# Jaureguy760/HaploHyped-VarAwareML

Hardware: AMD Instinct MI355X
Metric: variants/sec encode+compress, 3M-variant x 2.5k-sample VCF (higher is better)
Workload: dtype u8

## Files before the change

haplohyped_varawareml_amd/csrc/api.hip:

```cpp
#include "common.h"
#include <chrono>
#include <vector>
#include <stdarg.h>
#include <stdio.h>
#include <string.h>
#include <stdlib.h>

static thread_local char g_err[512] = "";

void hhgt_set_error(const char *fmt, ...)
{
    va_list ap;
    va_start(ap, fmt);
    vsnprintf(g_err, sizeof(g_err), fmt, ap);
    va_end(ap);
}

extern "C" const char *hhgt_last_error(void) { return g_err; }
extern "C" const char *hhgt_version(void) { return "hhgt 0.1 (gfx950)"; }

extern "C" int hhgt_device_count(void)
{
    int n = 0;
    if (hipGetDeviceCount(&n) != hipSuccess) return 0;
    return n;
}

int DevBuf::ensure(size_t bytes)
{
    if (bytes <= cap) return HHGT_OK;
    if (p) {
        hipFree(p);
        p = nullptr;
        cap = 0;
    }
    size_t want = bytes + bytes / 8 + 256;
    static const bool dbg = getenv("HHGT_ALLOC_DEBUG") != nullptr;
    const auto t0 = std::chrono::steady_clock::now();
    hipError_t e = hipMalloc(&p, want);
    if (dbg)
        fprintf(stderr, "[alloc] %.3f ms  hipMalloc %zu took %.3f ms\n", std::chrono::duration<double>(t0.time_since_epoch()).count() * 1e3,
                want, std::chrono::duration<double>(std::chrono::steady_clock::now() - t0).count() * 1e3);
    if (e != hipSuccess) {
        p = nullptr;
        hhgt_set_error("hipMalloc(%zu) failed: %s", want, hipGetErrorString(e));
        return HHGT_ERR_HIP;
    }
    cap = want;
    return HHGT_OK;
}

void DevBuf::release()
{
    if (p) hipFree(p);
    p = nullptr;
    cap = 0;
}

#define TRY(expr)                      \
    do {                               \
        int _rc = (expr);              \
        if (_rc != HHGT_OK) return _rc; \
    } while (0)

extern "C" int hhgt_ctx_create(int device, hhgt_ctx **out)
{
    if (!out) return HHGT_ERR_ARG;
    *out = nullptr;
    int n = hhgt_device_count();
    if (n <= 0 || device < 0 || device >= n) {
        hhgt_set_error("no usable HIP device (count=%d, requested=%d): libhhgt has no CPU path", n, device);
        return HHGT_ERR_NO_DEVICE;
    }
    HIP_TRY(hipSetDevice(device));
    hhgt_ctx *c = new hhgt_ctx();
    c->device = device;
    int rc = HHGT_OK;
    hipError_t e = hipGetDeviceProperties(&c->prop, device);
    if (e != hipSuccess) {
        hhgt_set_error("hipGetDeviceProperties failed: %s", hipGetErrorString(e));
        rc = HHGT_ERR_HIP;
    } else if (strncmp(c->prop.gcnArchName, "gfx950", 6) != 0) {
        hhgt_set_error("device %d is %s; libhhgt carries gfx950 code objects only", device, c->prop.gcnArchName);
        rc = HHGT_ERR_NO_DEVICE;
    }
    if (rc == HHGT_OK && (e = hipHostMalloc(reinterpret_cast<void **>(&c->h_counters), sizeof(DevCounters), hipHostMallocDefault)) != hipSuccess) {
        hhgt_set_error("hipHostMalloc failed: %s", hipGetErrorString(e));
        rc = HHGT_ERR_HIP;
    }
    if (rc == HHGT_OK && (e = hipHostMalloc(reinterpret_cast<void **>(&c->h_result_pinned), sizeof(hhgt_encode_result), hipHostMallocDefault)) != hipSuccess) {
        hhgt_set_error("hipHostMalloc failed: %s", hipGetErrorString(e));
        rc = HHGT_ERR_HIP;
    }
    if (rc == HHGT_OK) rc = c->counters.ensure(sizeof(DevCounters));
    if (rc != HHGT_OK) {
        hhgt_ctx_destroy(c);
        return rc;
    }
    *out = c;
    return HHGT_OK;
}

extern "C" void hhgt_ctx_destroy(hhgt_ctx *c)
{
    if (!c) return;
    hipSetDevice(c->device);
    hipDeviceSynchronize();
    DevBuf *bufs[] = {&c->slots, &c->counts, &c->prefix, &c->nl, &c->scan_tmp, &c->l_soff, &c->l_lend, &c->l_pos,
                      &c->l_refalt, &c->l_flags, &c->l_keep, &c->l_kidx, &c->l_cnew, &c->l_crun, &c->k_soff,
                      &c->k_lend, &c->k_meta, &c->redo_list, &c->redo_flag, &c->run_first, &c->run_names,
                      &c->counters, &c->cursor, &c->result, &c->dec_bad, &c->oh_ovl, &c->oh_lut, &c->crc_x2n};
    for (DevBuf *b : bufs) b->release();
    for (auto &w : c->cw) {
        DevBuf *wb[] = {&w.lz_scratch, &w.lz_csize, &w.lz_flags, &w.fr_bsize, &w.fr_csize, &w.fr_flags};
        for (DevBuf *b : wb) b->release();
        if (w.lz_done) hipEventDestroy(w.lz_done);
        if (w.fr_done) hipEventDestroy(w.fr_done);
    }
    if (c->h_counters) hipHostFree(c->h_counters);
    if (c->h_result_pinned) hipHostFree(c->h_result_pinned);
    for (auto &p : c->pending) {
        hipEventDestroy(p.a);
        hipEventDestroy(p.b);
    }
    for (auto e : c->event_pool) hipEventDestroy(e);
    delete c;
}

static hipEvent_t get_event(hhgt_ctx *c)
{
    if (!c->event_pool.empty()) {
        hipEvent_t e = c->event_pool.back();
        c->event_pool.pop_back();
        return e;
    }
    hipEvent_t e;
    hipEventCreate(&e);
    return e;
}

StageTimer::StageTimer(hhgt_ctx *c, hipStream_t s, int stage_) : ctx(c), st(s), stage(stage_)
{
    if (ctx->profiling) {
        a = get_event(ctx);
        b = get_event(ctx);
        hipEventRecord(a, st);
    }
}

void StageTimer::stop()
{
    if (a) {
        hipEventRecord(b, st);
        ctx->pending.push_back({stage, a, b});
        a = b = nullptr;
    }
}

int hhgt_profile_collect(hhgt_ctx *c)
{
    for (auto &p : c->pending) {
        hipEventSynchronize(p.b);
        float ms = 0.f;
        if (hipEventElapsedTime(&ms, p.a, p.b) == hipSuccess) {
            c->stage_ms[p.stage] += ms;
            c->stage_launches[p.stage] += 1;
        }
        c->event_pool.push_back(p.a);
        c->event_pool.push_back(p.b);
    }
    c->pending.clear();
    return HHGT_OK;
}

extern "C" int hhgt_profile_enable(hhgt_ctx *c, int on)
{
    if (!c) return HHGT_ERR_ARG;
    c->profiling = on ? 1 : 0;
    return HHGT_OK;
}

extern "C" int hhgt_profile_reset(hhgt_ctx *c)
{
    if (!c) return HHGT_ERR_ARG;
    hhgt_profile_collect(c);
    for (int i = 0; i < HHGT_N_STAGES; ++i) {
        c->stage_ms[i] = 0;
        c->stage_launches[i] = 0;
    }
    return HHGT_OK;
}

extern "C" int hhgt_profile_read(hhgt_ctx *c, double *ms, uint64_t *launches)
{
    if (!c) return HHGT_ERR_ARG;
    hhgt_profile_collect(c);
    for (int i = 0; i < HHGT_N_STAGES; ++i) {
        if (ms) ms[i] = c->stage_ms[i];
        if (launches) launches[i] = c->stage_launches[i];
    }
    return HHGT_OK;
}

static int make_layout(const hhgt_layout *lay, LayoutDev *L)
{
    if (!lay || lay->n_samples < 0) {
        hhgt_set_error("layout: bad n_samples");
        return HHGT_ERR_ARG;
    }
    L->S = (uint32_t)lay->n_samples;
    L->v_capacity = lay->v_capacity;
    L->ring = 0;
    L->pad_ = 0;
    if (lay->ring < 0 || (lay->ring > 0 && (lay->vc <= 0 || lay->v_capacity != (uint64_t)lay->ring * (uint64_t)lay->vc))) {
        hhgt_set_error("layout: a ring needs vc > 0 and v_capacity == ring * vc");
        return HHGT_ERR_ARG;
    }
    L->ring = (uint32_t)lay->ring;
    if (lay->vc == 0) {
        L->Vc = lay->v_capacity ? lay->v_capacity : TILE_V;
    } else {
        L->Vc = (uint64_t)lay->vc;
    }
    if (L->Vc % TILE_V) {
        hhgt_set_error("layout: variants per chunk (%llu) must be a multiple of %d (dense: v_capacity)",
                       (unsigned long long)L->Vc, TILE_V);
        return HHGT_ERR_ARG;
    }
    if (lay->v_capacity % L->Vc) {
        hhgt_set_error("layout: v_capacity must be a multiple of vc");
        return HHGT_ERR_ARG;
    }
    if (lay->sc == 0) {
        L->Sc = L->S ? L->S : 1;
        L->sc_log2 = 31;
        L->n_sc = 1;
    } else {
        uint32_t sc = (uint32_t)lay->sc;
        if (sc & (sc - 1)) {
            hhgt_set_error("layout: sc must be a power of two");
            return HHGT_ERR_ARG;
        }
        L->Sc = sc;
        uint32_t lg = 0;
        while ((1u << lg) < sc) ++lg;
        L->sc_log2 = lg;
        L->n_sc = (L->S + sc - 1) / sc;
        if (L->n_sc == 0) L->n_sc = 1;
    }
    return HHGT_OK;
}

extern "C" uint64_t hhgt_layout_bytes(const hhgt_layout *lay)
{
    LayoutDev L;
    if (make_layout(lay, &L) != HHGT_OK) return 0;
    return (uint64_t)L.n_sc * L.Sc * L.v_capacity * 2ull;
}

extern "C" uint64_t hhgt_layout_offset(const hhgt_layout *lay, uint32_t s, uint64_t v)
{
    LayoutDev L;
    if (make_layout(lay, &L) != HHGT_OK) return ~0ull;
    return layout_offset(L, s, v);
}

static int parse_region_host(const char *region, RegionFilter *rf)
{
    memset(rf, 0, sizeof(*rf));
    if (!region || !*region) return HHGT_OK;
    const char *colon = strrchr(region, ':');
    size_t clen = strlen(region);
    if (colon && colon[1] >= '0' && colon[1] <= '9') {
        char *p;
        long long b = strtoll(colon + 1, &p, 10), e = 0x7fffffffffffffffLL;
        while (*p == ',') p++;
        if (*p == '-' && p[1]) e = strtoll(p + 1, &p, 10);
        clen = (size_t)(colon - region);
        rf->has_range = 1;
        rf->beg = b;
        rf->end = e;
    }
    if (clen == 0 || clen >= sizeof(rf->contig)) {
        hhgt_set_error("region '%s': contig name empty or longer than 63 bytes", region);
        return HHGT_ERR_ARG;
    }
    memcpy(rf->contig, region, clen);
    rf->contig_len = (int)clen;
    return HHGT_OK;
}

__global__ void k_encode_finish(DevCounters *cnt, uint64_t *cursor, const uint64_t *__restrict__ run_first,
                                const uint8_t *__restrict__ run_names, uint64_t v_capacity, hhgt_encode_result *res)
{
    const uint32_t t = threadIdx.x;
    const uint64_t before = *cursor;
    const uint64_t kept = cnt->n_kept;
    __syncthreads();
    if (t == 0) {
        *cursor = before + kept;
        cnt->cursor_after = before + kept;
        res->stats.n_lines = cnt->n_lines;
        res->stats.n_records = cnt->n_records;
        res->stats.n_kept = kept;
        res->stats.n_drop_region = cnt->n_drop_region;
        res->stats.n_drop_filter = cnt->n_drop_filter;
        res->stats.n_haploid_padded = cnt->n_haploid;
        res->stats.n_malformed = cnt->n_malformed;
        res->stats.n_general_lines = cnt->n_general;
        res->stats.n_chrom_runs = cnt->n_chrom_runs;
        res->cursor_before = before;
        res->cursor_after = before + kept;
        res->n_lines_over = cnt->err_lines;
        res->err_density = cnt->err_density;
        res->v_capacity = v_capacity;
        res->done = 1u;
        res->reserved = cnt->n_other > 0xFFFFFFFFull ? 0xFFFFFFFFu : (uint32_t)cnt->n_other;
    }
    const uint64_t n_runs = cnt->n_chrom_runs;
    if (t < HHGT_RESULT_RUNS) res->run_first[t] = t < n_runs ? run_first[t] : 0ull;
    for (uint32_t q = t; q < HHGT_RESULT_RUNS * 32u; q += blockDim.x)
        res->run_names[q >> 5][q & 31u] = (q >> 5) < n_runs ? (char)run_names[q] : 0;
    __syncthreads();
    if (t < sizeof(DevCounters) / 8u) reinterpret_cast<unsigned long long *>(cnt)[t] = 0ull;
}

__global__ void k_set_u64(uint64_t *p, uint64_t v) { *p = v; }

static int encode_check_args(hhgt_ctx *c, const void *d_text, uint64_t nbytes, const hhgt_layout *lay, LayoutDev *L,
                             const char *region, RegionFilter *rf, void *d_G)
{
    TRY(make_layout(lay, L));
    if (nbytes >= 0xFFFFFFF0ull) {
        hhgt_set_error("encode: text block of %llu bytes; split it below 4 GiB at a line boundary",
                       (unsigned long long)nbytes);
        return HHGT_ERR_ARG;
    }
    if (nbytes && (!d_text || (reinterpret_cast<uintptr_t>(d_text) & 15u))) {
        hhgt_set_error("encode: d_text must be a 16-byte aligned device pointer");
        return HHGT_ERR_ARG;
    }
    if (L->S > 0 && !d_G) {
        hhgt_set_error("encode: d_G is NULL");
        return HHGT_ERR_ARG;
    }
    const int rc = parse_region_host(region, rf);
    rf->keep_multi = c->keep_multi;
    return rc;
}

static int encode_stage_index(hhgt_ctx *c, const uint8_t *text, uint64_t nbytes, uint32_t n_regions, uint32_t min_line, uint32_t S,
                              DevCounters *cnt, hipStream_t st)
{
    TRY(c->slots.ensure((size_t)n_regions * INDEX_CAP * 4));
    TRY(c->counts.ensure((size_t)n_regions * 4));
    TRY(c->prefix.ensure(((size_t)n_regions + 1) * 4));
    TRY(c->scan_tmp.ensure(2 * scan_tmp_elems(n_regions) * 4));
    TRY(launch_index_newlines(text, nbytes, c->slots.as<uint32_t>(), c->counts.as<uint32_t>(), n_regions, min_line, S, c->index_mode, cnt, st));
    TRY(launch_scan_exclusive_u32_pair(c->counts.as<uint32_t>(), c->prefix.as<uint32_t>(), nullptr, nullptr, n_regions,
                                       c->scan_tmp.as<uint32_t>(), c->scan_tmp.cap / 4, st));
    return HHGT_OK;
}

static int encode_stage_rest(hhgt_ctx *c, const uint8_t *text, uint64_t nbytes, uint32_t n_regions, uint32_t max_lines,
                             const RegionFilter &rf, const LayoutDev &L, const uint64_t *d_cursor, void *d_G, void *d_P, uint32_t *d_start, uint32_t *d_stop,
                             uint8_t *d_ref, uint8_t *d_alt, DevCounters *cnt, hipStream_t st)
{
    const uint32_t *d_nlines = c->prefix.as<uint32_t>() + n_regions;
    const size_t nl4 = ((size_t)max_lines + 1) * 4;
    TRY(c->nl.ensure(nl4));
    TRY(c->scan_tmp.ensure(2 * scan_tmp_elems(max_lines) * 4));
    DevBuf *per_line[] = {&c->l_soff, &c->l_lend, &c->l_pos, &c->l_refalt, &c->l_flags, &c->l_keep,
                          &c->l_kidx, &c->l_cnew, &c->l_crun, &c->k_soff, &c->k_lend, &c->k_meta,
                          &c->redo_list, &c->redo_flag};
    for (DevBuf *b : per_line) TRY(b->ensure(nl4));
    TRY(c->run_first.ensure(MAX_CHROM_RUNS * 8));
    TRY(c->run_names.ensure(MAX_CHROM_RUNS * 32));
    {
        StageTimer t(c, st, HHGT_STAGE_INDEX);
        TRY(launch_compact_newlines(c->slots.as<uint32_t>(), c->counts.as<uint32_t>(), c->prefix.as<uint32_t>(),
                                    n_regions, c->nl.as<uint32_t>(), max_lines, st));
        t.stop();
    }
    if (max_lines == 0) return HHGT_OK;
    {
        StageTimer t(c, st, HHGT_STAGE_FIXED);
        TRY(launch_parse_fixed(text, nbytes, c->nl.as<uint32_t>(), d_nlines, max_lines, rf, L.S,
                               c->l_soff.as<uint32_t>(), c->l_lend.as<uint32_t>(), c->l_pos.as<uint32_t>(),
                               c->l_refalt.as<uint32_t>(), c->l_flags.as<uint32_t>(), c->l_keep.as<uint32_t>(),
                               c->l_cnew.as<uint32_t>(), c->index_mode, cnt, st));
        TRY(launch_scan_exclusive_u32_pair(c->l_keep.as<uint32_t>(), c->l_kidx.as<uint32_t>(), c->l_cnew.as<uint32_t>(),
                                           c->l_crun.as<uint32_t>(), max_lines, c->scan_tmp.as<uint32_t>(), c->scan_tmp.cap / 4, st));
        TRY(launch_compact_kept(text, nbytes, c->nl.as<uint32_t>(), d_nlines, max_lines, c->l_soff.as<uint32_t>(),
                                c->l_lend.as<uint32_t>(), c->l_pos.as<uint32_t>(), c->l_refalt.as<uint32_t>(),
                                c->l_flags.as<uint32_t>(), c->l_kidx.as<uint32_t>(), c->l_crun.as<uint32_t>(),
                                c->k_soff.as<uint32_t>(), c->k_lend.as<uint32_t>(), c->k_meta.as<uint32_t>(),
                                c->redo_list.as<uint32_t>(), c->redo_flag.as<uint32_t>(), c->run_first.as<uint64_t>(), c->run_names.as<uint8_t>(),
                                MAX_CHROM_RUNS, d_cursor, L.v_capacity, L.ring, d_start, d_stop, d_ref, d_alt, cnt, d_P != nullptr, st));
        t.stop();
    }
    if (L.S > 0) {
        StageTimer t(c, st, HHGT_STAGE_ENCODE);
        if (d_P)
            TRY(launch_encode_planes(text, nbytes, c->k_soff.as<uint32_t>(), c->k_meta.as<uint32_t>(), max_lines, d_cursor, L,
                                     static_cast<uint8_t *>(d_P), static_cast<int8_t *>(d_G), c->redo_list.as<uint32_t>(),
                                     c->redo_flag.as<uint32_t>(), cnt, st));
        else
            TRY(launch_encode_tiles(text, nbytes, c->k_soff.as<uint32_t>(), c->k_meta.as<uint32_t>(), max_lines, d_cursor,
                                    L, static_cast<int8_t *>(d_G), c->redo_list.as<uint32_t>(),
                                    c->redo_flag.as<uint32_t>(), cnt, st));
        t.stop();
        StageTimer t2(c, st, HHGT_STAGE_GENERAL);
        TRY(launch_encode_general(text, nbytes, c->k_soff.as<uint32_t>(), c->k_lend.as<uint32_t>(),
                                  c->k_meta.as<uint32_t>(), c->redo_list.as<uint32_t>(), d_cursor, L,
                                  static_cast<int8_t *>(d_G), static_cast<uint8_t *>(d_P), cnt, c->prop.multiProcessorCount, st));
        t2.stop();
    }
    return HHGT_OK;
}

static int encode_finish(hhgt_ctx *c, uint64_t *d_cursor, const LayoutDev &L, DevCounters *cnt, hipStream_t st)
{
    TRY(c->run_first.ensure(MAX_CHROM_RUNS * 8));
    TRY(c->run_names.ensure(MAX_CHROM_RUNS * 32));
    TRY(c->result.ensure(sizeof(hhgt_encode_result)));
    hipLaunchKernelGGL(k_encode_finish, dim3(1), dim3(256), 0, st, cnt, d_cursor, c->run_first.as<uint64_t>(),
                       c->run_names.as<uint8_t>(), L.ring ? 0ull : L.v_capacity, c->result.as<hhgt_encode_result>());
    HIP_TRY(hipGetLastError());
    return HHGT_OK;
}

extern "C" int hhgt_encode_result_status(const hhgt_encode_result *r)
{
    if (!r) return HHGT_ERR_ARG;
    if (!r->done) {
        hhgt_set_error("encode: the result record is not complete yet (synchronise the stream first)");
        return HHGT_ERR_ARG;
    }
    if (r->err_density) {
        hhgt_set_error("encode: more than %u newlines inside one %u-byte region (not VCF text)", INDEX_CAP, INDEX_REGION);
        return HHGT_ERR_LINE_DENSITY;
    }
    if (r->n_lines_over) {
        hhgt_set_error("encode: %llu lines beyond max_lines were not encoded", (unsigned long long)r->n_lines_over);
        return HHGT_ERR_CAPACITY;
    }
    if (r->stats.n_malformed) {
        hhgt_set_error("Error parsing VCF file: %llu malformed record(s) (too few columns, bad POS, FORMAT without GT)",
                       (unsigned long long)r->stats.n_malformed);
        return HHGT_ERR_MALFORMED;
    }
    if (r->v_capacity && r->cursor_after > r->v_capacity) {
        hhgt_set_error("encode: %llu kept records at v_base %llu exceed v_capacity %llu",
                       (unsigned long long)r->stats.n_kept, (unsigned long long)r->cursor_before,
                       (unsigned long long)r->v_capacity);
        return HHGT_ERR_CAPACITY;
    }
    if (r->stats.n_chrom_runs > MAX_CHROM_RUNS) {
        hhgt_set_error("encode: %llu CHROM runs in one text block, more than the limit of %u (a run starts at every change of CHROM "
                       "and behind every empty or header line)",
                       (unsigned long long)r->stats.n_chrom_runs, MAX_CHROM_RUNS);
        return HHGT_ERR_CAPACITY;
    }
    return HHGT_OK;
}

static void empty_result(hhgt_encode_result *r)
{
    memset(r, 0, sizeof(*r));
    r->done = 1u;
}

static int planes_check_layout(const LayoutDev &L)
{
    if (L.Vc % 4096ull) {
        hhgt_set_error("planes: variants per chunk (%llu; dense: v_capacity) must be a multiple of 4096", (unsigned long long)L.Vc);
        return HHGT_ERR_ARG;
    }
    return HHGT_OK;
}

extern "C" uint64_t hhgt_planes_bytes(const hhgt_layout *lay)
{
    LayoutDev L;
    if (make_layout(lay, &L) != HHGT_OK || planes_check_layout(L) != HHGT_OK) return 0;
    return (uint64_t)L.n_sc * L.Sc * L.v_capacity / 2ull;
}

static int planes_columns(const hhgt_layout *lay, uint32_t col0, uint32_t n_cols, LayoutDev *L, PlanesGeom *pg)
{
    TRY(make_layout(lay, L));
    TRY(planes_check_layout(*L));
    if ((uint64_t)col0 + n_cols > L->v_capacity / L->Vc) {
        hhgt_set_error("planes: columns [%u, %u) outside the layout's %llu", col0, col0 + n_cols, (unsigned long long)(L->v_capacity / L->Vc));
        return HHGT_ERR_ARG;
    }
    *pg = planes_geom(*L, col0);
    return HHGT_OK;
}

static int encode_async_impl(hhgt_ctx *c, const void *d_text, uint64_t nbytes, const char *region, const hhgt_layout *lay,
                             uint64_t *d_cursor, uint32_t max_lines, void *d_G, void *d_P, bool planes, uint32_t *d_start,
                             uint32_t *d_stop, uint8_t *d_ref, uint8_t *d_alt, hhgt_encode_result *h_result, void *stream)
{
    if (!c || !d_cursor) return HHGT_ERR_ARG;
    hipStream_t st = reinterpret_cast<hipStream_t>(stream);
    HIP_TRY(hipSetDevice(c->device));
    LayoutDev L;
    RegionFilter rf;
    TRY(encode_check_args(c, d_text, nbytes, lay, &L, region, &rf, planes ? d_P : d_G));
    if (planes) TRY(planes_check_layout(L));
    const uint8_t *text = static_cast<const uint8_t *>(d_text);
    DevCounters *cnt = c->counters.as<DevCounters>();
    if (!c->counters_clean) HIP_TRY(hipMemsetAsync(cnt, 0, sizeof(DevCounters), st));
    c->counters_clean = false;
    const uint32_t n_regions = (uint32_t)((nbytes + 1 + INDEX_REGION - 1) / INDEX_REGION);
    if (nbytes) {
        {
            StageTimer t(c, st, HHGT_STAGE_INDEX);
            TRY(encode_stage_index(c, text, nbytes, n_regions, L.S ? 2u * L.S + 17u : 0u, L.S, cnt, st));
            t.stop();
        }
        TRY(encode_stage_rest(c, text, nbytes, n_regions, max_lines, rf, L, d_cursor, d_G, planes ? d_P : nullptr, d_start, d_stop, d_ref,
                              d_alt, cnt, st));
    }
    TRY(encode_finish(c, d_cursor, L, cnt, st));
    c->counters_clean = true;
    if (h_result) {
        h_result->done = 0u;
        HIP_TRY(hipMemcpyAsync(h_result, c->result.p, sizeof(hhgt_encode_result), hipMemcpyDeviceToHost, st));
    }
    return HHGT_OK;
}

extern "C" int hhgt_encode_text_async(hhgt_ctx *c, const void *d_text, uint64_t nbytes, const char *region,
                                      const hhgt_layout *lay, uint64_t *d_cursor, uint32_t max_lines, void *d_G,
                                      uint32_t *d_start, uint32_t *d_stop, uint8_t *d_ref, uint8_t *d_alt,
                                      hhgt_encode_result *h_result, void *stream)
{
    return encode_async_impl(c, d_text, nbytes, region, lay, d_cursor, max_lines, d_G, nullptr, false, d_start, d_stop, d_ref, d_alt,
                             h_result, stream);
}

extern "C" int hhgt_encode_text_planes_async(hhgt_ctx *c, const void *d_text, uint64_t nbytes, const char *region,
                                             const hhgt_layout *lay, uint64_t *d_cursor, uint32_t max_lines, void *d_P, void *d_G,
                                             uint32_t *d_start, uint32_t *d_stop, uint8_t *d_ref, uint8_t *d_alt,
                                             hhgt_encode_result *h_result, void *stream)
{
    return encode_async_impl(c, d_text, nbytes, region, lay, d_cursor, max_lines, d_G, d_P, true, d_start, d_stop, d_ref, d_alt,
                             h_result, stream);
}

extern "C" int hhgt_pad_tail_planes(hhgt_ctx *c, const hhgt_layout *lay, uint64_t v_end, uint64_t vcol_begin, uint64_t vcol_end,
                                    void *d_P, void *stream)
{
    if (!c || !d_P) return HHGT_ERR_ARG;
    HIP_TRY(hipSetDevice(c->device));
    LayoutDev L;
    TRY(make_layout(lay, &L));
    TRY(planes_check_layout(L));
    if (v_end > L.v_capacity || vcol_end > L.v_capacity / L.Vc) {
        hhgt_set_error("pad_tail: range outside the layout");
        return HHGT_ERR_ARG;
    }
    return launch_pad_tail_planes(L, v_end, vcol_begin, vcol_end, static_cast<uint8_t *>(d_P), reinterpret_cast<hipStream_t>(stream));
}

extern "C" int hhgt_pad_tail_planes_cursor(hhgt_ctx *c, const hhgt_layout *lay, const uint64_t *d_cursor, void *d_P, void *stream)
{
    if (!c || !d_P || !d_cursor) return HHGT_ERR_ARG;
    HIP_TRY(hipSetDevice(c->device));
    LayoutDev L;
    TRY(make_layout(lay, &L));
    TRY(planes_check_layout(L));
    return launch_pad_tail_planes_cursor(L, d_cursor, static_cast<uint8_t *>(d_P), reinterpret_cast<hipStream_t>(stream));
}

extern "C" int hhgt_planes_expand(hhgt_ctx *c, const hhgt_layout *lay, const void *d_P, const void *d_G, uint32_t col0, uint32_t n_cols,
                                  void *d_out, void *stream)
{
    if (!c || !d_P || !d_out) return HHGT_ERR_ARG;
    HIP_TRY(hipSetDevice(c->device));
    LayoutDev L;
    PlanesGeom pg;
    TRY(planes_columns(lay, col0, n_cols, &L, &pg));
    if (n_cols == 0) return HHGT_OK;
    return launch_planes_expand(L, static_cast<const uint8_t *>(d_P), static_cast<const uint8_t *>(d_G), col0, n_cols,
                                static_cast<uint8_t *>(d_out), reinterpret_cast<hipStream_t>(stream));
}

static int encode_text_once(hhgt_ctx *c, const void *d_text, uint64_t nbytes, const char *region, const hhgt_layout *lay, uint64_t v_base,
                            void *d_G, uint32_t *d_start, uint32_t *d_stop, uint8_t *d_ref, uint8_t *d_alt, hhgt_encode_stats *stats,
                            void *stream);

extern "C" int hhgt_encode_text(hhgt_ctx *c, const void *d_text, uint64_t nbytes, const char *region,
                                const hhgt_layout *lay, uint64_t v_base, void *d_G, uint32_t *d_start,
                                uint32_t *d_stop, uint8_t *d_ref, uint8_t *d_alt, hhgt_encode_stats *stats,
                                void *stream)
{
    int rc = encode_text_once(c, d_text, nbytes, region, lay, v_base, d_G, d_start, d_stop, d_ref, d_alt, stats, stream);
    if (rc == HHGT_ERR_MALFORMED && c && lay && lay->n_samples >= 760) {
        const int mode = c->index_mode < 0 ? index_mode_default() : c->index_mode;
        if (mode > 0) {
            const int saved = c->index_mode;
            c->index_mode = 0;
            rc = encode_text_once(c, d_text, nbytes, region, lay, v_base, d_G, d_start, d_stop, d_ref, d_alt, stats, stream);
            c->index_mode = saved;
        }
    }
    return rc;
}

static int encode_text_once(hhgt_ctx *c, const void *d_text, uint64_t nbytes, const char *region, const hhgt_layout *lay, uint64_t v_base,
                            void *d_G, uint32_t *d_start, uint32_t *d_stop, uint8_t *d_ref, uint8_t *d_alt, hhgt_encode_stats *stats,
                            void *stream)
{
    if (!c) return HHGT_ERR_ARG;
    hipStream_t st = reinterpret_cast<hipStream_t>(stream);
    HIP_TRY(hipSetDevice(c->device));
    if (stats) memset(stats, 0, sizeof(*stats));
    LayoutDev L;
    RegionFilter rf;
    TRY(encode_check_args(c, d_text, nbytes, lay, &L, region, &rf, d_G));
    c->run_first_kept.clear();
    c->run_names_host.clear();
    if (nbytes == 0) return HHGT_OK;

    const uint8_t *text = static_cast<const uint8_t *>(d_text);
    DevCounters *cnt = c->counters.as<DevCounters>();
    TRY(c->cursor.ensure(8));
    HIP_TRY(hipMemsetAsync(cnt, 0, sizeof(DevCounters), st));
    c->counters_clean = false;
    hipLaunchKernelGGL(k_set_u64, dim3(1), dim3(1), 0, st, c->cursor.as<uint64_t>(), v_base);
    const uint32_t n_regions = (uint32_t)((nbytes + 1 + INDEX_REGION - 1) / INDEX_REGION);
    uint32_t n_lines = 0;
    {
        StageTimer t(c, st, HHGT_STAGE_INDEX);
        TRY(encode_stage_index(c, text, nbytes, n_regions, L.S ? 2u * L.S + 17u : 0u, L.S, cnt, st));
        c->h_counters->n_lines = 0;
        c->h_counters->err_density = 0;
        HIP_TRY(hipMemcpyAsync(&c->h_counters->n_lines, c->prefix.as<uint32_t>() + n_regions, 4,
                               hipMemcpyDeviceToHost, st));
        HIP_TRY(hipMemcpyAsync(&c->h_counters->err_density, &cnt->err_density, 8, hipMemcpyDeviceToHost, st));
        HIP_TRY(hipStreamSynchronize(st));
        t.stop();
        n_lines = (uint32_t)(c->h_counters->n_lines & 0xFFFFFFFFull);
        if (c->h_counters->err_density) {
            hhgt_set_error("encode: more than %u newlines inside one %u-byte region (not VCF text)", INDEX_CAP,
                           INDEX_REGION);
            return HHGT_ERR_LINE_DENSITY;
        }
    }
    if (stats) stats->n_lines = n_lines;
    if (n_lines == 0) return HHGT_OK;
    TRY(encode_stage_rest(c, text, nbytes, n_regions, n_lines, rf, L, c->cursor.as<uint64_t>(), d_G, nullptr, d_start, d_stop, d_ref,
                          d_alt, cnt, st));
    TRY(encode_finish(c, c->cursor.as<uint64_t>(), L, cnt, st));
    c->counters_clean = true;
    hhgt_encode_result *hr = &c->h_result;
    hr->done = 0u;
    HIP_TRY(hipMemcpyAsync(c->h_result_pinned, c->result.p, sizeof(hhgt_encode_result), hipMemcpyDeviceToHost, st));
    HIP_TRY(hipStreamSynchronize(st));
    *hr = *c->h_result_pinned;
    if (stats) *stats = hr->stats;
    TRY(hhgt_encode_result_status(hr));
    const uint32_t n_runs = (uint32_t)hr->stats.n_chrom_runs;
    if (n_runs) {
        std::vector<uint64_t> first(n_runs);
        std::vector<char> names((size_t)n_runs * 32);
        if (n_runs <= HHGT_RESULT_RUNS) {
            memcpy(first.data(), hr->run_first, n_runs * 8);
            memcpy(names.data(), hr->run_names, (size_t)n_runs * 32);
        } else {
            HIP_TRY(hipMemcpy(first.data(), c->run_first.p, (size_t)n_runs * 8, hipMemcpyDeviceToHost));
            HIP_TRY(hipMemcpy(names.data(), c->run_names.p, (size_t)n_runs * 32, hipMemcpyDeviceToHost));
        }
        for (uint32_t r = 0; r < n_runs; ++r) {
            c->run_first_kept.push_back(first[r]);
            c->run_names_host.emplace_back(names.data() + (size_t)r * 32, strnlen(names.data() + (size_t)r * 32, 31));
        }
    }
    return HHGT_OK;
}

extern "C" int hhgt_encode_chrom_runs(hhgt_ctx *c, uint32_t max_runs, uint64_t *first_kept, char *names,
                                      uint32_t *n_runs)
{
    if (!c || !n_runs) return HHGT_ERR_ARG;
    uint32_t n = (uint32_t)c->run_first_kept.size();
    *n_runs = n;
    if (n > max_runs) n = max_runs;
    for (uint32_t r = 0; r < n; ++r) {
        if (first_kept) first_kept[r] = c->run_first_kept[r];
        if (names) {
            memset(names + (size_t)r * 32, 0, 32);
            size_t l = c->run_names_host[r].size() < 31 ? c->run_names_host[r].size() : 31;
            memcpy(names + (size_t)r * 32, c->run_names_host[r].data(), l);
        }
    }
    return HHGT_OK;
}

extern "C" int hhgt_pad_tail(hhgt_ctx *c, const hhgt_layout *lay, uint64_t v_end, uint64_t vcol_begin,
                             uint64_t vcol_end, void *d_G, void *stream)
{
    if (!c || !d_G) return HHGT_ERR_ARG;
    HIP_TRY(hipSetDevice(c->device));
    LayoutDev L;
    TRY(make_layout(lay, &L));
    if (v_end > L.v_capacity || vcol_end > L.v_capacity / L.Vc) {
        hhgt_set_error("pad_tail: range outside the layout");
        return HHGT_ERR_ARG;
    }
    return launch_pad_tail(L, v_end, vcol_begin, vcol_end, static_cast<int8_t *>(d_G),
                           reinterpret_cast<hipStream_t>(stream));
}

extern "C" int hhgt_pad_tail_cursor(hhgt_ctx *c, const hhgt_layout *lay, const uint64_t *d_cursor, void *d_G, void *stream)
{
    if (!c || !d_G || !d_cursor) return HHGT_ERR_ARG;
    HIP_TRY(hipSetDevice(c->device));
    LayoutDev L;
    TRY(make_layout(lay, &L));
    return launch_pad_tail_cursor(L, d_cursor, static_cast<int8_t *>(d_G), reinterpret_cast<hipStream_t>(stream));
}

static int check_codec_args(uint64_t chunk_nbytes, int typesize, int blocksize, int format)
{
    if (typesize < 1 || typesize > 255 || blocksize < 16 || blocksize > 65536 || blocksize % typesize ||
        chunk_nbytes == 0 || chunk_nbytes >= 0x7fffffffull || (format != HHGT_BLOSC1 && format != HHGT_BLOSC2)) {
        hhgt_set_error("compress: bad arguments (chunk_nbytes=%llu typesize=%d blocksize=%d format=%d)",
                       (unsigned long long)chunk_nbytes, typesize, blocksize, format);
        return HHGT_ERR_ARG;
    }
    return HHGT_OK;
}

static int effective_blocksize(uint64_t chunk_nbytes, int typesize, int blocksize)
{
    if ((uint64_t)blocksize > chunk_nbytes) {
        blocksize = (int)chunk_nbytes;
        if (typesize > 1 && blocksize >= typesize) blocksize -= blocksize % typesize;
    }
    return blocksize > 0 ? blocksize : 1;
}

static int check_decode_block(int typesize, int blocksize)
{
    if (blocksize > 65536) {
        hhgt_set_error("decode: block of %d bytes x typesize %d does not fit LDS (blocks of at most 65536 bytes)",
                       blocksize, typesize);
        return HHGT_ERR_ARG;
    }
    return HHGT_OK;
}

static void codec_geometry(uint64_t chunk_nbytes, int typesize, int blocksize, uint32_t *nblocks, uint32_t *nwaves,
                           size_t *slot_bytes)
{
    const bool split = typesize >= 2 && typesize <= 16 && blocksize / typesize >= 128;
    *nblocks = (uint32_t)((chunk_nbytes + blocksize - 1) / blocksize);
    *nwaves = split ? (uint32_t)typesize : 1u;
    size_t max_stream = split ? (size_t)blocksize / typesize : (size_t)blocksize;
    if (split && chunk_nbytes % blocksize && chunk_nbytes % blocksize > max_stream) max_stream = chunk_nbytes % blocksize;
    *slot_bytes = lz4_slot_bytes((int)max_stream);
}

extern "C" uint64_t hhgt_compress_bound(uint64_t n_chunks, uint64_t chunk_nbytes, int typesize, int blocksize)
{
    if (check_codec_args(chunk_nbytes, typesize, blocksize, HHGT_BLOSC2) != HHGT_OK) return 0;
    return n_chunks * (chunk_nbytes + 32);
}

static int compress_impl(hhgt_ctx *c, const void *d_src, const void *d_planes, PlanesGeom pg, uint64_t n_chunks, uint64_t chunk_nbytes,
                         int typesize, int blocksize, int format, void *d_dst, uint64_t dst_cap,
                         uint64_t *d_chunk_off, uint64_t *total_bytes, void *stream)
{
    if (!c || (!d_src && !d_planes) || !d_dst || !d_chunk_off) return HHGT_ERR_ARG;
    hipStream_t st = reinterpret_cast<hipStream_t>(stream);
    HIP_TRY(hipSetDevice(c->device));
    TRY(check_codec_args(chunk_nbytes, typesize, blocksize, format));
    if (total_bytes) *total_bytes = 0;
    if (n_chunks == 0) return HHGT_OK;
    if (!total_bytes && dst_cap < n_chunks * (chunk_nbytes + 32)) {
        hhgt_set_error("compress: the asynchronous form (total_bytes == NULL) needs dst_cap >= hhgt_compress_bound() = %llu, got %llu",
                       (unsigned long long)(n_chunks * (chunk_nbytes + 32)), (unsigned long long)dst_cap);
        return HHGT_ERR_CAPACITY;
    }
    blocksize = effective_blocksize(chunk_nbytes, typesize, blocksize);
    uint32_t nblocks, nwaves;
    size_t slot;
    codec_geometry(chunk_nbytes, typesize, blocksize, &nblocks, &nwaves, &slot);
    const uint64_t n_streams = n_chunks * nblocks * nwaves;
    hipStream_t fst = c->frame_stream ? c->frame_stream : st;
    hhgt_ctx::CodecWs &w = c->cw[c->frame_stream ? (c->cmp_seq++ & 1u) : 0u];
    TRY(w.lz_scratch.ensure((size_t)n_streams * slot));
    TRY(w.lz_csize.ensure((size_t)n_streams * 4));
    TRY(w.fr_bsize.ensure((size_t)n_chunks * nblocks * 4));
    TRY(w.fr_csize.ensure(((size_t)n_chunks + 1) * 8));
    TRY(w.fr_flags.ensure((size_t)n_chunks * 4));
    if (w.fr_pending) {
        HIP_TRY(hipStreamWaitEvent(st, w.fr_done, 0));
        w.fr_pending = false;
    }
    {
        StageTimer t(c, st, HHGT_STAGE_LZ4);
        if (!w.lz_flags.p) {
            TRY(w.lz_flags.ensure(4));
            HIP_TRY(hipMemsetAsync(w.lz_flags.p, 0, 4, st));
        }
        if (++w.lz_tag == 0) w.lz_tag = 1;
        TRY(launch_lz4_blocks(static_cast<const uint8_t *>(d_src), static_cast<const uint8_t *>(d_planes), pg, n_chunks, chunk_nbytes, typesize,
                              blocksize, w.lz_scratch.as<uint8_t>(), slot, w.lz_csize.as<uint32_t>(), c->clevel, w.lz_flags.as<uint32_t>(),
                              w.lz_tag, st));
        t.stop();
    }
    if (fst != st) {
        if (!w.lz_done) HIP_TRY(hipEventCreateWithFlags(&w.lz_done, hipEventDisableTiming));
        if (!w.fr_done) HIP_TRY(hipEventCreateWithFlags(&w.fr_done, hipEventDisableTiming));
        HIP_TRY(hipEventRecord(w.lz_done, st));
        HIP_TRY(hipStreamWaitEvent(fst, w.lz_done, 0));
    }
    {
        StageTimer t(c, fst, HHGT_STAGE_FRAME);
        TRY(launch_frame(w.lz_scratch.as<uint8_t>(), slot, w.lz_csize.as<uint32_t>(),
                         static_cast<const uint8_t *>(d_src), static_cast<const uint8_t *>(d_planes), pg, n_chunks, chunk_nbytes, typesize,
                         blocksize, format, w.fr_bsize.as<uint32_t>(), w.fr_csize.as<uint64_t>(), static_cast<uint8_t *>(d_dst),
                         dst_cap, d_chunk_off, w.fr_flags.as<uint32_t>(), fst));
        t.stop();
    }
    if (fst != st) {
        HIP_TRY(hipEventRecord(w.fr_done, fst));
        w.fr_pending = true;
        if (total_bytes) HIP_TRY(hipStreamWaitEvent(st, w.fr_done, 0));
    }
    if (total_bytes) {
        uint64_t tot = 0;
        HIP_TRY(hipMemcpyAsync(&tot, d_chunk_off + n_chunks, 8, hipMemcpyDeviceToHost, st));
        HIP_TRY(hipStreamSynchronize(st));
        *total_bytes = tot;
        if (tot > dst_cap) {
            hhgt_set_error("compress: need %llu bytes, dst_cap is %llu", (unsigned long long)tot,
                           (unsigned long long)dst_cap);
            return HHGT_ERR_CAPACITY;
        }
    }
    return HHGT_OK;
}

extern "C" int hhgt_compress_chunks(hhgt_ctx *c, const void *d_src, uint64_t n_chunks, uint64_t chunk_nbytes,
                                    int typesize, int blocksize, int format, void *d_dst, uint64_t dst_cap,
                                    uint64_t *d_chunk_off, uint64_t *total_bytes, void *stream)
{
    if (!d_src) return HHGT_ERR_ARG;
    return compress_impl(c, d_src, nullptr, PlanesGeom{0, 0, 0, 0}, n_chunks, chunk_nbytes, typesize, blocksize, format, d_dst, dst_cap,
                         d_chunk_off, total_bytes, stream);
}

extern "C" int hhgt_compress_planes(hhgt_ctx *c, const hhgt_layout *lay, const void *d_P, const void *d_G, uint32_t col0, uint32_t n_cols,
                                    int format, void *d_dst, uint64_t dst_cap, uint64_t *d_chunk_off, uint64_t *total_bytes,
                                    void *stream)
{
    if (!c || !d_P) return HHGT_ERR_ARG;
    LayoutDev L;
    PlanesGeom pg;
    TRY(planes_columns(lay, col0, n_cols, &L, &pg));
    const uint64_t chunk_nbytes = (uint64_t)L.Sc * L.Vc * 2ull, col_bytes = chunk_nbytes * L.n_sc;
    const uint8_t *g = d_G ? static_cast<const uint8_t *>(d_G) + (uint64_t)col0 * col_bytes : nullptr;
    return compress_impl(c, g, d_P, pg, (uint64_t)n_cols * L.n_sc, chunk_nbytes, 2, 8192, format, d_dst, dst_cap, d_chunk_off, total_bytes,
                         stream);
}

extern "C" int hhgt_reserve(hhgt_ctx *c, uint64_t text_bytes, uint32_t max_lines, uint64_t n_chunks, uint64_t chunk_nbytes, int typesize,
                            int blocksize)
{
    if (!c) return HHGT_ERR_ARG;
    HIP_TRY(hipSetDevice(c->device));
    if (text_bytes) {
        const uint32_t n_regions = (uint32_t)((text_bytes + 1 + INDEX_REGION - 1) / INDEX_REGION);
        TRY(c->slots.ensure((size_t)n_regions * INDEX_CAP * 4));
        TRY(c->counts.ensure((size_t)n_regions * 4));
        TRY(c->prefix.ensure(((size_t)n_regions + 1) * 4));
        const size_t st_el = scan_tmp_elems(n_regions) > scan_tmp_elems(max_lines) ? scan_tmp_elems(n_regions) : scan_tmp_elems(max_lines);
        TRY(c->scan_tmp.ensure(2 * st_el * 4));
        const size_t nl4 = ((size_t)max_lines + 1) * 4;
        TRY(c->nl.ensure(nl4));
        DevBuf *per_line[] = {&c->l_soff, &c->l_lend, &c->l_pos, &c->l_refalt, &c->l_flags, &c->l_keep, &c->l_kidx, &c->l_cnew, &c->l_crun,
                              &c->k_soff, &c->k_lend, &c->k_meta, &c->redo_list, &c->redo_flag};
        for (DevBuf *b : per_line) TRY(b->ensure(nl4));
        TRY(c->run_first.ensure(MAX_CHROM_RUNS * 8));
        TRY(c->run_names.ensure(MAX_CHROM_RUNS * 32));
        TRY(c->result.ensure(sizeof(hhgt_encode_result)));
    }
    if (n_chunks) {
        TRY(check_codec_args(chunk_nbytes, typesize, blocksize, HHGT_BLOSC2));
        blocksize = effective_blocksize(chunk_nbytes, typesize, blocksize);
        uint32_t nblocks, nwaves;
        size_t slot;
        codec_geometry(chunk_nbytes, typesize, blocksize, &nblocks, &nwaves, &slot);
        const uint64_t n_streams = n_chunks * nblocks * nwaves;
        hhgt_ctx::CodecWs &w = c->cw[0];
        TRY(w.lz_scratch.ensure((size_t)n_streams * slot));
        TRY(w.lz_csize.ensure((size_t)n_streams * 4));
        TRY(w.fr_bsize.ensure((size_t)n_chunks * nblocks * 4));
        TRY(w.fr_csize.ensure(((size_t)n_chunks + 1) * 8));
        TRY(w.fr_flags.ensure((size_t)n_chunks * 4));
    }
    return HHGT_OK;
}

extern "C" int hhgt_set_clevel(hhgt_ctx *c, int clevel)
{
    if (!c || clevel < 1 || clevel > 9) {
        hhgt_set_error("clevel must be 1..9");
        return HHGT_ERR_ARG;
    }
    c->clevel = clevel;
    return HHGT_OK;
}

extern "C" int hhgt_stream_create(hhgt_ctx *c, int kind, void **out)
{
    if (!c || !out || (kind != HHGT_STREAM_ENCODE && kind != HHGT_STREAM_COMPRESS && kind != HHGT_STREAM_FRAME)) {
        hhgt_set_error("hhgt_stream_create: bad arguments");
        return HHGT_ERR_ARG;
    }
    HIP_TRY(hipSetDevice(c->device));
    hipStream_t st = nullptr;
    if (kind == HHGT_STREAM_FRAME) {
        HIP_TRY(hipStreamCreateWithFlags(&st, hipStreamNonBlocking));
    } else if (kind == HHGT_STREAM_ENCODE) {
        int lo = 0, hi = 0;
        HIP_TRY(hipDeviceGetStreamPriorityRange(&lo, &hi));
        HIP_TRY(hipStreamCreateWithPriority(&st, hipStreamNonBlocking, hi));
    } else {
        const uint32_t n_cu = (uint32_t)c->prop.multiProcessorCount;
        uint32_t use = n_cu >= 128u ? (n_cu * 3u / 4u) / 32u * 32u : n_cu;
        if (const char *e = getenv("HHGT_COMPRESS_CUS")) {
            const int v = atoi(e);
            use = v <= 0 || (uint32_t)v >= n_cu ? n_cu : (uint32_t)v;
        }
        if (use >= n_cu) {
            HIP_TRY(hipStreamCreateWithFlags(&st, hipStreamNonBlocking));
        } else {
            std::vector<uint32_t> mask((n_cu + 31u) / 32u, 0u);
            for (uint32_t i = n_cu - use; i < n_cu; ++i) mask[i >> 5] |= 1u << (i & 31u);
            if (hipExtStreamCreateWithCUMask(&st, (uint32_t)mask.size(), mask.data()) != hipSuccess) {
                (void)hipGetLastError();
                st = nullptr;
                HIP_TRY(hipStreamCreateWithFlags(&st, hipStreamNonBlocking));
            }
        }
    }
    *out = st;
    return HHGT_OK;
}

extern "C" int hhgt_set_frame_stream(hhgt_ctx *c, void *stream)
{
    if (!c) return HHGT_ERR_ARG;
    HIP_TRY(hipSetDevice(c->device));
    if (c->frame_stream) HIP_TRY(hipStreamSynchronize(c->frame_stream));
    for (auto &w : c->cw) w.fr_pending = false;
    c->frame_stream = reinterpret_cast<hipStream_t>(stream);
    return HHGT_OK;
}

extern "C" int hhgt_stream_destroy(hhgt_ctx *c, void *stream)
{
    if (!c) return HHGT_ERR_ARG;
    if (stream) {
        HIP_TRY(hipSetDevice(c->device));
        if (reinterpret_cast<hipStream_t>(stream) == c->frame_stream) TRY(hhgt_set_frame_stream(c, nullptr));
        HIP_TRY(hipStreamDestroy(reinterpret_cast<hipStream_t>(stream)));
    }
    return HHGT_OK;
}

extern "C" int hhgt_set_index_mode(hhgt_ctx *c, int mode)
{
    if (!c || mode < -1 || mode > 2) {
        hhgt_set_error("index mode must be -1 (default), 0 (scan), 1 (hop) or 2 (walk)");
        return HHGT_ERR_ARG;
    }
    c->index_mode = mode;
    return HHGT_OK;
}

extern "C" int hhgt_set_keep_multiallelic(hhgt_ctx *c, int on)
{
    if (!c) return HHGT_ERR_ARG;
    c->keep_multi = on ? 1 : 0;
    return HHGT_OK;
}

__global__ void k_count_nonzero_u32(const uint32_t *__restrict__ v, uint64_t n, unsigned long long *out)
{
    uint64_t i = (uint64_t)blockIdx.x * blockDim.x + threadIdx.x;
    const unsigned long long m = __ballot(i < n && v[i] != 0u);
    if ((threadIdx.x & 63u) == 0u && m) atomicAdd(out, (unsigned long long)__builtin_popcountll(m));
}

extern "C" int hhgt_inflate_members(hhgt_ctx *c, const void *d_src, uint64_t src_bytes, const uint64_t *d_comp_off,
                                    const uint32_t *d_comp_len, const uint64_t *d_out_off, const uint32_t *d_isize,
                                    uint64_t n_members, void *d_dst, uint64_t dst_bytes, const uint32_t *d_crc32,
                                    uint32_t *d_status, uint64_t *n_bad, void *stream)
{
    if (!c || !d_src || !d_comp_off || !d_comp_len || !d_out_off || !d_isize || !d_status || (!d_dst && dst_bytes))
        return HHGT_ERR_ARG;
    hipStream_t st = reinterpret_cast<hipStream_t>(stream);
    HIP_TRY(hipSetDevice(c->device));
    if (n_bad) *n_bad = 0;
    if (n_members == 0) return HHGT_OK;
    if (d_crc32 && !c->crc_x2n_ready) {
        uint32_t t[32];
        crc32_x2n_table(t);
        TRY(c->crc_x2n.ensure(sizeof(t)));
        HIP_TRY(hipMemcpy(c->crc_x2n.p, t, sizeof(t), hipMemcpyHostToDevice));
        c->crc_x2n_ready = true;
    }
    {
        StageTimer t(c, st, HHGT_STAGE_INFLATE);
        TRY(launch_inflate(static_cast<const uint8_t *>(d_src), src_bytes, d_comp_off, d_comp_len, d_out_off, d_isize,
                           n_members, static_cast<uint8_t *>(d_dst), dst_bytes, d_status, d_crc32,
                           c->crc_x2n.as<uint32_t>(), st));
        t.stop();
    }
    if (n_bad) {
        TRY(c->dec_bad.ensure(8));
        HIP_TRY(hipMemsetAsync(c->dec_bad.p, 0, 8, st));
        hipLaunchKernelGGL(k_count_nonzero_u32, dim3((uint32_t)((n_members + 255) / 256)), dim3(256), 0, st, d_status,
                           n_members, c->dec_bad.as<unsigned long long>());
        HIP_TRY(hipGetLastError());
        uint64_t nb = 0;
        HIP_TRY(hipMemcpyAsync(&nb, c->dec_bad.p, 8, hipMemcpyDeviceToHost, st));
        HIP_TRY(hipStreamSynchronize(st));
        *n_bad = nb;
    }
    return HHGT_OK;
}

extern "C" int hhgt_decompress_chunks(hhgt_ctx *c, const void *d_src, const uint64_t *d_chunk_off, uint64_t n_chunks,
                                      uint64_t chunk_nbytes, int typesize, int blocksize, void *d_dst,
                                      uint64_t *n_bad, void *stream)
{
    if (!c || !d_src || !d_dst || !d_chunk_off) return HHGT_ERR_ARG;
    hipStream_t st = reinterpret_cast<hipStream_t>(stream);
    HIP_TRY(hipSetDevice(c->device));
    TRY(check_decode_block(typesize, blocksize));
    TRY(check_codec_args(chunk_nbytes, typesize, blocksize, HHGT_BLOSC2));
    if (n_bad) *n_bad = 0;
    if (n_chunks == 0) return HHGT_OK;
    blocksize = effective_blocksize(chunk_nbytes, typesize, blocksize);
    TRY(c->dec_bad.ensure(8));
    HIP_TRY(hipMemsetAsync(c->dec_bad.p, 0, 8, st));
    {
        StageTimer t(c, st, HHGT_STAGE_DECODE);
        TRY(launch_decode(static_cast<const uint8_t *>(d_src), d_chunk_off, n_chunks, chunk_nbytes, typesize,
                          blocksize, static_cast<uint8_t *>(d_dst), c->dec_bad.as<unsigned long long>(), st));
        t.stop();
    }
    if (n_bad) {
        uint64_t nb = 0;
        HIP_TRY(hipMemcpyAsync(&nb, c->dec_bad.p, 8, hipMemcpyDeviceToHost, st));
        HIP_TRY(hipStreamSynchronize(st));
        *n_bad = nb;
    }
    return HHGT_OK;
}

extern "C" int hhgt_decompress_blocks(hhgt_ctx *c, const hhgt_block_sel *d_sel, uint32_t n_sel, uint64_t chunk_nbytes,
                                      int typesize, int blocksize, void *d_dst, uint64_t *n_bad, void *stream)
{
    if (!c || (n_sel && (!d_sel || !d_dst))) {
        hhgt_set_error("decompress_blocks: null %s", !c ? "context" : !d_sel ? "selection array" : "destination");
        return HHGT_ERR_ARG;
    }
    hipStream_t st = reinterpret_cast<hipStream_t>(stream);
    HIP_TRY(hipSetDevice(c->device));
    TRY(check_decode_block(typesize, blocksize));
    TRY(check_codec_args(chunk_nbytes, typesize, blocksize, HHGT_BLOSC2));
    if (n_bad) *n_bad = 0;
    if (n_sel == 0) return HHGT_OK;
    blocksize = effective_blocksize(chunk_nbytes, typesize, blocksize);
    TRY(c->dec_bad.ensure(8));
    HIP_TRY(hipMemsetAsync(c->dec_bad.p, 0, 8, st));
    {
        StageTimer t(c, st, HHGT_STAGE_DECODE);
        TRY(launch_decode_sel(d_sel, n_sel, chunk_nbytes, typesize, blocksize, static_cast<uint8_t *>(d_dst),
                              c->dec_bad.as<unsigned long long>(), st));
        t.stop();
    }
    if (n_bad) {
        uint64_t nb = 0;
        HIP_TRY(hipMemcpyAsync(&nb, c->dec_bad.p, 8, hipMemcpyDeviceToHost, st));
        HIP_TRY(hipStreamSynchronize(st));
        *n_bad = nb;
    }
    return HHGT_OK;
}

extern "C" int hhgt_count_alleles(hhgt_ctx *c, const hhgt_count_sel *d_sel, uint32_t n_sel, uint32_t sc, uint32_t vc,
                                  int typesize, int blocksize, uint32_t *d_counts, uint64_t n_out, uint64_t *n_bad,
                                  void *stream)
{
    if (!c || (n_sel && (!d_sel || !d_counts))) {
        hhgt_set_error("count_alleles: null %s", !c ? "context" : !d_sel ? "selection array" : "counts");
        return HHGT_ERR_ARG;
    }
    if (typesize != 2) {
        hhgt_set_error("count_alleles: typesize %d (only 2: one diploid int8 call)", typesize);
        return HHGT_ERR_ARG;
    }
    if (sc < 1 || sc > 64 || vc < 1) {
        hhgt_set_error("count_alleles: chunk of %u samples x %u variants (1 to 64 samples)", sc, vc);
        return HHGT_ERR_ARG;
    }
    const uint64_t chunk_nbytes = (uint64_t)sc * vc * 2u;
    TRY(check_codec_args(chunk_nbytes, typesize, blocksize, HHGT_BLOSC2));
    if (blocksize > 8192 || ((uint64_t)vc * 2u) % (uint64_t)blocksize) {
        hhgt_set_error("count_alleles: blocksize %d does not cut a row of %u variants into whole blocks of at most 8192 "
                       "bytes", blocksize, vc);
        return HHGT_ERR_ARG;
    }
    hipStream_t st = reinterpret_cast<hipStream_t>(stream);
    HIP_TRY(hipSetDevice(c->device));
    if (n_bad) *n_bad = 0;
    if (n_sel == 0) return HHGT_OK;
    TRY(c->dec_bad.ensure(8));
    HIP_TRY(hipMemsetAsync(c->dec_bad.p, 0, 8, st));
    {
        StageTimer t(c, st, HHGT_STAGE_DECODE);
        TRY(launch_count_alleles(d_sel, n_sel, sc, vc, blocksize, d_counts, n_out, c->dec_bad.as<unsigned long long>(), st));
        t.stop();
    }
    if (n_bad) {
        uint64_t nb = 0;
        HIP_TRY(hipMemcpyAsync(&nb, c->dec_bad.p, 8, hipMemcpyDeviceToHost, st));
        HIP_TRY(hipStreamSynchronize(st));
        *n_bad = nb;
    }
    return HHGT_OK;
}

extern "C" int hhgt_count_samples(hhgt_ctx *c, const hhgt_sample_sel *d_sel, uint32_t n_sel, uint32_t sc, uint32_t vc,
                                  int typesize, int blocksize, const uint32_t *d_vmask, uint64_t vmask_words,
                                  uint32_t *d_counts, uint64_t n_out, uint64_t *n_bad, void *stream)
{
    if (!c || (n_sel && (!d_sel || !d_counts))) {
        hhgt_set_error("count_samples: null %s", !c ? "context" : !d_sel ? "selection array" : "counts");
        return HHGT_ERR_ARG;
    }
    if (typesize != 2) {
        hhgt_set_error("count_samples: typesize %d (only 2: one diploid int8 call)", typesize);
        return HHGT_ERR_ARG;
    }
    if (sc < 1 || sc > 64 || vc < 1) {
        hhgt_set_error("count_samples: chunk of %u samples x %u variants (1 to 64 samples)", sc, vc);
        return HHGT_ERR_ARG;
    }
    const uint64_t chunk_nbytes = (uint64_t)sc * vc * 2u;
    TRY(check_codec_args(chunk_nbytes, typesize, blocksize, HHGT_BLOSC2));
    if (blocksize > 8192 || ((uint64_t)vc * 2u) % (uint64_t)blocksize) {
        hhgt_set_error("count_samples: blocksize %d does not cut a row of %u variants into whole blocks of at most 8192 "
                       "bytes", blocksize, vc);
        return HHGT_ERR_ARG;
    }
    hipStream_t st = reinterpret_cast<hipStream_t>(stream);
    HIP_TRY(hipSetDevice(c->device));
    if (n_bad) *n_bad = 0;
    if (n_sel == 0) return HHGT_OK;
    TRY(c->dec_bad.ensure(8));
    HIP_TRY(hipMemsetAsync(c->dec_bad.p, 0, 8, st));
    {
        StageTimer t(c, st, HHGT_STAGE_DECODE);
        TRY(launch_count_samples(d_sel, n_sel, sc, vc, blocksize, d_vmask, vmask_words, d_counts, n_out,
                                 c->dec_bad.as<unsigned long long>(), st));
        t.stop();
    }
    if (n_bad) {
        uint64_t nb = 0;
        HIP_TRY(hipMemcpyAsync(&nb, c->dec_bad.p, 8, hipMemcpyDeviceToHost, st));
        HIP_TRY(hipStreamSynchronize(st));
        *n_bad = nb;
    }
    return HHGT_OK;
}
```

haplohyped_varawareml_amd/csrc/common.h:

```cpp
#pragma once
#include <hip/hip_runtime.h>
#include <stdint.h>
#include <stddef.h>
#include <string>
#include <vector>
#include "../../include/hhgt.h"

#define HHGT_WAVE 64
#ifdef HHGT_ENC_PRIO
#define HHGT_WAVE_PRIO() __builtin_amdgcn_s_setprio(HHGT_ENC_PRIO)
#else
#define HHGT_WAVE_PRIO()
#endif

#ifdef __HIPCC__
__device__ __forceinline__ uint32_t wave_scan_sum_dpp(uint32_t x, uint32_t lane)
{
    x += (uint32_t)__builtin_amdgcn_update_dpp(0, (int)x, 0x111, 0xf, 0xf, false);
    x += (uint32_t)__builtin_amdgcn_update_dpp(0, (int)x, 0x112, 0xf, 0xf, false);
    x += (uint32_t)__builtin_amdgcn_update_dpp(0, (int)x, 0x114, 0xf, 0xf, false);
    x += (uint32_t)__builtin_amdgcn_update_dpp(0, (int)x, 0x118, 0xf, 0xf, false);
    const uint32_t t0 = (uint32_t)__builtin_amdgcn_readlane((int)x, 15);
    const uint32_t t1 = (uint32_t)__builtin_amdgcn_readlane((int)x, 31) + t0;
    const uint32_t t2 = (uint32_t)__builtin_amdgcn_readlane((int)x, 47) + t1;
    const uint32_t row = lane >> 4;
    return x + (row == 0u ? 0u : (row == 1u ? t0 : (row == 2u ? t1 : t2)));
}
#endif

void hhgt_set_error(const char *fmt, ...);
#define HIP_TRY(expr)                                                                      \
    do {                                                                                   \
        hipError_t _e = (expr);                                                            \
        if (_e != hipSuccess) {                                                            \
            hhgt_set_error("%s failed: %s (%s:%d)", #expr, hipGetErrorString(_e), __FILE__, \
                           __LINE__);                                                      \
            return HHGT_ERR_HIP;                                                           \
        }                                                                                  \
    } while (0)

enum : uint32_t {
    LF_RECORD = 1u,
    LF_KEEP = 2u,
    LF_FAST = 4u,
    LF_MALFORMED = 8u,
    LF_DROP_REGION = 16u,
    LF_DROP_FILTER = 32u,
    LF_CHROM_NEW = 64u,
};

struct DevCounters {
    unsigned long long n_lines;
    unsigned long long n_records;
    unsigned long long n_kept;
    unsigned long long n_drop_region;
    unsigned long long n_drop_filter;
    unsigned long long n_haploid;
    unsigned long long n_malformed;
    unsigned long long n_general;
    unsigned long long n_chrom_runs;
    unsigned long long err_density;
    unsigned long long err_lines;
    unsigned long long cursor_after;
    unsigned long long n_other;
    unsigned long long pad[3];
};

#define MAX_CHROM_RUNS 4096u

struct RegionFilter {
    char contig[64];
    int contig_len;
    int has_range;
    long long beg, end;
    int keep_multi;
};

#define INDEX_REGION 16384u
#define INDEX_CAP 1024u

#define TILE_V 128
#define TILE_S 256

struct LayoutDev {
    uint32_t S;
    uint32_t sc_log2;
    uint32_t n_sc;
    uint32_t Sc;
    uint64_t Vc;
    uint64_t v_capacity;
    uint32_t ring;
    uint32_t pad_;
};

#define PL_TILE 256u
struct PlanesGeom {
    uint32_t S_pad;
    uint32_t bpr;
    uint32_t tpc;
    uint32_t col0;
};
static inline __host__ __device__ uint64_t planes_piece(const PlanesGeom &g, uint64_t col, uint32_t tile, uint32_t kp, uint32_t row)
{
    return ((((col * g.tpc + tile) * 4ull + kp) * g.S_pad) + row) * 32ull;
}
static inline __host__ __device__ PlanesGeom planes_geom(const LayoutDev &L, uint32_t col0)
{
    PlanesGeom g;
    g.S_pad = L.n_sc * L.Sc;
    g.bpr = (uint32_t)(L.Vc >> 12);
    g.tpc = (uint32_t)(L.Vc / PL_TILE);
    g.col0 = col0;
    return g;
}
static inline __host__ __device__ void planes_block(const PlanesGeom &g, uint64_t id, uint64_t *col, uint32_t *row, uint32_t *bi)
{
    const uint64_t per_col = (uint64_t)g.S_pad * g.bpr;
    const uint64_t c = id / per_col;
    const uint32_t rem = (uint32_t)(id - c * per_col);
    *col = g.col0 + c;
    *row = rem / g.bpr;
    *bi = rem - (rem / g.bpr) * g.bpr;
}

struct DevBuf {
    void *p = nullptr;
    size_t cap = 0;
    int ensure(size_t bytes);
    void release();
    template <typename T> T *as() const { return reinterpret_cast<T *>(p); }
};

struct hhgt_ctx {
    int device = 0;
    hipDeviceProp_t prop;
    DevBuf slots, counts, prefix, nl, scan_tmp;
    DevBuf l_soff, l_lend, l_pos, l_refalt, l_flags, l_keep, l_kidx, l_cnew, l_crun;
    DevBuf k_soff, k_lend, k_meta, redo_list, redo_flag, run_first, run_names;
    DevBuf counters;
    DevBuf cursor;
    DevBuf result;
    struct CodecWs {
        DevBuf lz_scratch, lz_csize, lz_flags, fr_bsize, fr_csize, fr_flags;
        uint32_t lz_tag = 0;
        hipEvent_t lz_done = nullptr, fr_done = nullptr;
        bool fr_pending = false;
    } cw[2];
    uint64_t cmp_seq = 0;
    hipStream_t frame_stream = nullptr;
    DevBuf dec_bad, oh_ovl, oh_lut, crc_x2n;
    bool crc_x2n_ready = false;
    DevCounters *h_counters = nullptr;
    hhgt_encode_result *h_result_pinned = nullptr;
    hhgt_encode_result h_result;
    std::vector<uint64_t> run_first_kept;
    std::vector<std::string> run_names_host;
    int clevel = 5;
    int keep_multi = 0;
    int index_mode = -1;
    bool counters_clean = false;
    int profiling = 0;
    double stage_ms[HHGT_N_STAGES] = {0};
    uint64_t stage_launches[HHGT_N_STAGES] = {0};
    struct Pending { int stage; hipEvent_t a, b; };
    std::vector<Pending> pending;
    std::vector<hipEvent_t> event_pool;
};

struct StageTimer {
    hhgt_ctx *ctx;
    hipStream_t st;
    int stage;
    hipEvent_t a = nullptr, b = nullptr;
    StageTimer(hhgt_ctx *c, hipStream_t s, int stage_);
    void stop();
};
int hhgt_profile_collect(hhgt_ctx *ctx);

int launch_scan_exclusive_u32(const uint32_t *d_in, uint32_t *d_out, uint64_t n, uint32_t *d_tmp,
                              size_t tmp_elems, hipStream_t st);
int launch_scan_exclusive_u32_pair(const uint32_t *in_a, uint32_t *out_a, const uint32_t *in_b, uint32_t *out_b, uint64_t n,
                                   uint32_t *d_tmp, size_t tmp_elems, hipStream_t st);
size_t scan_tmp_elems(uint64_t n);

int launch_index_newlines(const uint8_t *d_text, uint64_t n, uint32_t *d_slots, uint32_t *d_counts,
                          uint32_t n_regions, uint32_t min_line, uint32_t S, int mode, DevCounters *d_cnt, hipStream_t st);
int index_mode_default();
int launch_compact_newlines(const uint32_t *d_slots, const uint32_t *d_counts, const uint32_t *d_prefix,
                            uint32_t n_regions, uint32_t *d_nl, uint32_t max_lines, hipStream_t st);
int launch_parse_fixed(const uint8_t *d_text, uint64_t n, const uint32_t *d_nl, const uint32_t *d_nlines,
                       uint32_t max_lines, const RegionFilter &region, uint32_t S, uint32_t *l_soff, uint32_t *l_lend,
                       uint32_t *l_pos, uint32_t *l_refalt, uint32_t *l_flags, uint32_t *l_keep,
                       uint32_t *l_cnew, int mode, DevCounters *d_cnt, hipStream_t st);
int launch_compact_kept(const uint8_t *d_text, uint64_t n, const uint32_t *d_nl, const uint32_t *d_nlines, uint32_t max_lines,
                        const uint32_t *l_soff, const uint32_t *l_lend,
                        const uint32_t *l_pos, const uint32_t *l_refalt, const uint32_t *l_flags,
                        const uint32_t *l_kidx, const uint32_t *l_crun, uint32_t *k_soff, uint32_t *k_lend,
                        uint32_t *k_meta, uint32_t *redo_list, uint32_t *redo_flag, uint64_t *run_first, uint8_t *run_names,
                        uint32_t max_runs, const uint64_t *d_cursor, uint64_t v_capacity, uint32_t ring, uint32_t *d_start,
                        uint32_t *d_stop, uint8_t *d_ref, uint8_t *d_alt, DevCounters *d_cnt, bool strided, hipStream_t st);

int launch_encode_tiles(const uint8_t *d_text, uint64_t n, const uint32_t *k_soff, const uint32_t *k_meta,
                        uint32_t n_lines_bound, const uint64_t *d_cursor, LayoutDev lay, int8_t *d_G,
                        uint32_t *redo_list, uint32_t *redo_flag, DevCounters *d_cnt, hipStream_t st);
int launch_encode_general(const uint8_t *d_text, uint64_t n, const uint32_t *k_soff, const uint32_t *k_lend,
                          const uint32_t *k_meta, const uint32_t *redo_list, const uint64_t *d_cursor, LayoutDev lay,
                          int8_t *d_G, uint8_t *d_P, DevCounters *d_cnt, int n_cu, hipStream_t st);
int launch_encode_planes(const uint8_t *d_text, uint64_t n, const uint32_t *k_soff, const uint32_t *k_meta,
                         uint32_t n_lines_bound, const uint64_t *d_cursor, LayoutDev lay, uint8_t *d_P, int8_t *d_G,
                         uint32_t *redo_list, uint32_t *redo_flag, DevCounters *d_cnt, hipStream_t st);
int launch_pad_tail_planes(LayoutDev lay, uint64_t v_end, uint64_t vcol_begin, uint64_t vcol_end, uint8_t *d_P, hipStream_t st);
int launch_pad_tail_planes_cursor(LayoutDev lay, const uint64_t *d_cursor, uint8_t *d_P, hipStream_t st);
int launch_planes_expand(LayoutDev lay, const uint8_t *d_P, const uint8_t *d_G, uint32_t col0, uint32_t n_cols, uint8_t *d_out, hipStream_t st);
int launch_pad_tail(LayoutDev lay, uint64_t v_end, uint64_t vcol_begin, uint64_t vcol_end, int8_t *d_G,
                    hipStream_t st);
int launch_pad_tail_cursor(LayoutDev lay, const uint64_t *d_cursor, int8_t *d_G, hipStream_t st);

size_t lz4_slot_bytes(int neblock);
int launch_lz4_blocks(const uint8_t *d_src, const uint8_t *d_planes, PlanesGeom pg, uint64_t n_chunks, uint64_t chunk_nbytes, int typesize,
                      int blocksize, uint8_t *d_scratch, size_t slot_bytes, uint32_t *d_csize, int clevel, uint32_t *d_flags, uint32_t tag,
                      hipStream_t st);
int launch_lz4_bitplanes(const uint8_t *d_src, bool planes, PlanesGeom pg, uint64_t n_blocks, uint8_t *d_scratch, size_t slot_bytes, uint32_t *d_csize,
                         int depth, uint32_t *d_flags, uint32_t tag, hipStream_t st);
int launch_frame(const uint8_t *d_scratch, size_t slot_bytes, const uint32_t *d_csize, const uint8_t *d_src, const uint8_t *d_planes,
                 PlanesGeom pg, uint64_t n_chunks, uint64_t chunk_nbytes, int typesize, int blocksize, int format,
                 uint32_t *d_bstart, uint64_t *d_chunk_csize, uint8_t *d_dst, uint64_t dst_cap,
                 uint64_t *d_chunk_off, uint32_t *d_chunk_flags, hipStream_t st);
int launch_decode(const uint8_t *d_src, const uint64_t *d_chunk_off, uint64_t n_chunks, uint64_t chunk_nbytes,
                  int typesize, int blocksize, uint8_t *d_dst, unsigned long long *d_bad, hipStream_t st);
int launch_decode_sel(const hhgt_block_sel *d_sel, uint32_t n_sel, uint64_t chunk_nbytes, int typesize, int blocksize,
                      uint8_t *d_dst, unsigned long long *d_bad, hipStream_t st);
int launch_count_alleles(const hhgt_count_sel *d_sel, uint32_t n_sel, uint32_t sc, uint32_t vc, int blocksize,
                         uint32_t *d_counts, uint64_t n_out, unsigned long long *d_bad, hipStream_t st);
int launch_count_samples(const hhgt_sample_sel *d_sel, uint32_t n_sel, uint32_t sc, uint32_t vc, int blocksize,
                         const uint32_t *d_vmask, uint64_t vmask_words, uint32_t *d_counts, uint64_t n_out,
                         unsigned long long *d_bad, hipStream_t st);
int launch_inflate(const uint8_t *d_src, uint64_t src_bytes, const uint64_t *d_comp_off, const uint32_t *d_comp_len,
                   const uint64_t *d_out_off, const uint32_t *d_isize, uint64_t n_members, uint8_t *d_dst,
                   uint64_t dst_bytes, uint32_t *d_status, const uint32_t *d_crc32, const uint32_t *d_x2n, hipStream_t st);
void crc32_x2n_table(uint32_t *t );

static inline __host__ __device__ uint64_t layout_offset(const LayoutDev &L, uint32_t s, uint64_t v)
{
    uint64_t vcol = v / L.Vc, vin = v - vcol * L.Vc;
    if (L.ring) vcol %= L.ring;
    uint32_t scol = (L.sc_log2 >= 31) ? 0u : (s >> L.sc_log2);
    uint32_t sin = s - scol * L.Sc;
    return (((vcol * L.n_sc + scol) * L.Sc + sin) * L.Vc + vin) * 2ull;
}
```

haplohyped_varawareml_amd/csrc/index.hip:

```cpp
#include "common.h"

typedef uint32_t u32x4_unaligned __attribute__((ext_vector_type(4), aligned(1)));
typedef uint32_t u32x4_t __attribute__((ext_vector_type(4)));

__device__ __forceinline__ uint32_t nl_mask4(uint32_t x)
{
    uint32_t t = x ^ 0x0A0A0A0Au;
    uint32_t z = ~(((t & 0x7F7F7F7Fu) + 0x7F7F7F7Fu) | t | 0x7F7F7F7Fu);
    return (((z >> 7) * 0x01020408u) >> 24) & 0xFu;
}

__global__ __launch_bounds__(256) void k_index_newlines(const uint8_t *__restrict__ text, uint64_t n,
                                                        uint32_t *__restrict__ slots,
                                                        uint32_t *__restrict__ counts, uint32_t n_regions,
                                                        DevCounters *cnt)
{
    HHGT_WAVE_PRIO();
    const uint32_t lane = threadIdx.x & 63u;
    const uint32_t r = blockIdx.x * 4u + (threadIdx.x >> 6);
    if (r >= n_regions) return;
    const bool virt = n > 0 && text[n - 1] != '\n';
    const uint64_t rbase = (uint64_t)r * INDEX_REGION;
    uint32_t *my = slots + (size_t)r * INDEX_CAP;
    uint32_t wcount = 0;
    bool overflow = false;
    uint32_t masks[INDEX_REGION / 1024];
#pragma unroll
    for (int it = 0; it < (int)(INDEX_REGION / 1024); ++it) {
        uint64_t g0 = rbase + (uint64_t)it * 1024u + lane * 16u;
        uint32_t m = 0;
        if (g0 + 16 <= n) {
            const u32x4_t v4 = __builtin_nontemporal_load(reinterpret_cast<const u32x4_t *>(text + g0));
            uint4 v = make_uint4(v4.x, v4.y, v4.z, v4.w);
            m = nl_mask4(v.x) | (nl_mask4(v.y) << 4) | (nl_mask4(v.z) << 8) | (nl_mask4(v.w) << 12);
        } else if (g0 <= n) {
            for (int j = 0; j < 16; ++j) {
                uint64_t g = g0 + j;
                if (g < n) {
                    if (text[g] == '\n') m |= 1u << j;
                } else if (g == n && virt)
                    m |= 1u << j;
            }
        }
        masks[it] = m;
    }
#pragma unroll
    for (int it = 0; it < (int)(INDEX_REGION / 1024); ++it) {
        uint32_t m = masks[it];
        if (__ballot(m != 0) == 0ull) continue;
        uint32_t c = __popc(m);
        uint32_t inc = c;
#pragma unroll
        for (int d = 1; d < 64; d <<= 1) {
            uint32_t t = __shfl_up(inc, d, 64);
            if (lane >= (uint32_t)d) inc += t;
        }
        uint32_t idx = wcount + inc - c;
        uint32_t g0 = (uint32_t)(rbase + (uint64_t)it * 1024u + lane * 16u);
        while (m) {
            int j = __ffs(m) - 1;
            m &= m - 1;
            if (idx < INDEX_CAP) my[idx] = g0 + (uint32_t)j;
            else overflow = true;
            ++idx;
        }
        wcount += __shfl(inc, 63, 64);
    }
    if (__ballot(overflow) != 0ull && lane == 0) atomicAdd(&cnt->err_density, 1ull);
    if (lane == 0) counts[r] = wcount < INDEX_CAP ? wcount : INDEX_CAP;
}

__device__ __forceinline__ uint32_t eq_mask4(uint32_t x, uint32_t c4)
{
    const uint32_t t = x ^ c4;
    const uint32_t z = ~(((t & 0x7F7F7F7Fu) + 0x7F7F7F7Fu) | t | 0x7F7F7F7Fu);
    return (((z >> 7) * 0x01020408u) >> 24) & 0xFu;
}

__device__ __forceinline__ uint32_t eq_mask16(const u32x4_t &v, uint32_t c4)
{
    return eq_mask4(v.x, c4) | (eq_mask4(v.y, c4) << 4) | (eq_mask4(v.z, c4) << 8) | (eq_mask4(v.w, c4) << 12);
}

__device__ __forceinline__ uint32_t head_byte(const u32x4_t &v, uint32_t off)
{
    const uint32_t q = (off >> 2) & 3u;
    const uint32_t d = q == 0u ? v.x : (q == 1u ? v.y : (q == 2u ? v.z : v.w));
    return ((uint32_t)__builtin_amdgcn_readlane((int)d, (int)(off >> 4)) >> (8u * (off & 3u))) & 0xFFu;
}

__device__ __forceinline__ uint32_t head_kth(uint32_t m16, uint32_t cum, uint32_t k)
{
    const unsigned long long b = __builtin_amdgcn_ballot_w64(cum < k && cum + (uint32_t)__popc(m16) >= k);
    const int l = __builtin_ctzll(b);
    uint32_t m = (uint32_t)__builtin_amdgcn_readlane((int)m16, l);
    const uint32_t r = k - (uint32_t)__builtin_amdgcn_readlane((int)cum, l);
    for (uint32_t i = 1; i < r; ++i) m &= m - 1u;
    return 16u * (uint32_t)l + (uint32_t)__builtin_ctz(m);
}

#ifndef WALK_BATCH
#define WALK_BATCH 1
#endif
#ifndef WALK_PF
#define WALK_PF 0
#endif
template <int U, bool WALK>
__global__ __launch_bounds__(256) void k_index_hop(const uint8_t *__restrict__ text, uint64_t n, uint32_t *__restrict__ slots,
                                                   uint32_t *__restrict__ counts, uint32_t n_regions, uint32_t skip, uint32_t S,
                                                   DevCounters *cnt, uint32_t HOP_K)
{
    HHGT_WAVE_PRIO();
    const uint32_t lane = threadIdx.x & 63u;
    const uint32_t w = (uint32_t)__builtin_amdgcn_readfirstlane((int)(blockIdx.x * 4u + (threadIdx.x >> 6)));
    const uint32_t r_first = w * HOP_K;
    if (r_first >= n_regions) return;
    const uint32_t r_cnt = n_regions - r_first < HOP_K ? n_regions - r_first : HOP_K;
    const bool virt = n > 0 && text[n - 1] != '\n';
    const uint64_t beg = (uint64_t)r_first * INDEX_REGION;
    uint64_t endw = beg + (uint64_t)r_cnt * INDEX_REGION;
    if (endw > n + 1) endw = n + 1;
    const uint64_t last_term = virt ? n : n - 1;
    uint32_t cntv = 0;
    bool overflow = false;
    uint64_t pos = beg;
    uint64_t cand = 0, fb = 0;
    bool have_cand = false;
    uint64_t est_len = 0, pf_wb = 0;
    bool pf_valid = false;
    u32x4_t pf = u32x4_t{0u, 0u, 0u, 0u};
    auto record = [&](uint64_t q) {
        const uint32_t rr = (uint32_t)(q / INDEX_REGION), local = rr - r_first;
        const uint32_t c = (uint32_t)__builtin_amdgcn_readlane((int)cntv, (int)local);
        if (c < INDEX_CAP) {
            if (lane == 0) slots[(size_t)rr * INDEX_CAP + c] = (uint32_t)q;
        } else
            overflow = true;
        cntv += lane == local ? 1u : 0u;
    };
    bool no_batch = false, bat_off = false;
    uint32_t bat_fail = 0;
    uint64_t head_p = 0;
    bool cand_batch = false;
    bool rehead = false;
    while (have_cand || pos < endw) {
        if (WALK && WALK_BATCH && have_cand && !no_batch && !bat_off && est_len != 0ull && cand >= 40ull && cand + 3ull * est_len + 216ull <= n) {
            const uint32_t g = lane >> 4, li = lane & 15u;
            const uint64_t L0 = est_len;
            const uint8_t *wbase = text + (cand - 40ull);
            const uint64_t voff = (uint64_t)g * L0 + 16ull * li;
            const u32x4_t v = *reinterpret_cast<const u32x4_unaligned *>(wbase + voff);
            const uint32_t nlm = eq_mask16(v, 0x0A0A0A0Au), tbm = eq_mask16(v, 0x09090909u);
            const unsigned long long nlb = __builtin_amdgcn_ballot_w64(nlm != 0u);
            uint32_t og[4];
            bool vg[4];
#pragma unroll
            for (int k = 0; k < 4; ++k) {
                const uint32_t mg = (uint32_t)(nlb >> (16 * k)) & 0xFFFFu;
                vg[k] = mg != 0u;
                const int fl = 16 * k + __builtin_ctz(mg | 0x10000u);
                og[k] = 16u * ((uint32_t)fl & 15u) + (uint32_t)__builtin_ctz((uint32_t)__builtin_amdgcn_readlane((int)nlm, fl & 63) | 0x10000u);
            }
            const uint32_t o = g == 0u ? og[0] : (g == 1u ? og[1] : (g == 2u ? og[2] : og[3]));
            const uint32_t l0 = 16u * li;
            const uint32_t keep = l0 > o ? 0xFFFFu : (l0 + 15u <= o ? 0u : (0xFFFFu << (o - l0 + 1u)) & 0xFFFFu);
            const unsigned long long nl2 = __builtin_amdgcn_ballot_w64((nlm & keep) != 0u);
            const uint32_t tk = tbm & keep, tc = (uint32_t)__popc(tk);
            uint32_t incl = tc;
            incl += (uint32_t)__builtin_amdgcn_update_dpp(0, (int)incl, 0x111, 0xf, 0xf, false);
            incl += (uint32_t)__builtin_amdgcn_update_dpp(0, (int)incl, 0x112, 0xf, 0xf, false);
            incl += (uint32_t)__builtin_amdgcn_update_dpp(0, (int)incl, 0x114, 0xf, 0xf, false);
            incl += (uint32_t)__builtin_amdgcn_update_dpp(0, (int)incl, 0x118, 0xf, 0xf, false);
            const uint32_t cum = incl - tc;
            const bool has9 = cum < 9u && incl >= 9u;
            uint32_t m9 = tk;
            const uint32_t r1 = 8u - cum;
#pragma unroll
            for (uint32_t i = 0; i < 8u; ++i) m9 = i < r1 ? (m9 & (m9 - 1u)) : m9;
            const uint32_t j9 = (uint32_t)__builtin_ctz(m9 | 0x10000u) & 15u;
            const uint32_t pw = (uint32_t)__builtin_amdgcn_update_dpp(0, (int)v.w, 0x111, 0xf, 0xf, false);
            const uint32_t ptb = (uint32_t)__builtin_amdgcn_update_dpp(0, (int)tbm, 0x111, 0xf, 0xf, false);
            const uint32_t tb20 = (tbm << 4) | (ptb >> 12);
            const bool tab8 = ((tb20 >> (j9 + 1u)) & 1u) != 0u;
            const uint32_t ix = j9 + 2u, di = ix >> 2;
            const uint32_t w0 = di == 0u ? pw : (di == 1u ? v.x : (di == 2u ? v.y : (di == 3u ? v.z : v.w)));
            const uint32_t w1 = di == 0u ? v.x : (di == 1u ? v.y : (di == 2u ? v.z : v.w));
            const uint32_t gt2 = __builtin_amdgcn_alignbyte(w1, w0, ix & 3u) & 0xFFFFu;
            const bool ok9 = has9 && tab8 && gt2 == 0x5447u;
            const uint32_t t9 = l0 + j9;
            const unsigned long long b9 = __builtin_amdgcn_ballot_w64(ok9);
            uint64_t expected = cand, fbx = fb, exp_head = head_p;
            bool exp_batch = cand_batch;
            bool stop = false, handed = false;
            uint32_t advanced = 0;
#pragma unroll
            for (int k = 0; k < 4; ++k) {
                if (stop || handed) continue;
                const uint64_t nlpos = cand - 40ull + (uint64_t)k * L0 + og[k];
                const bool cr = vg[k] && og[k] != 0u && head_byte(v, 256u * (uint32_t)k + og[k] - 1u) == '\r';
                if (!vg[k] || nlpos != expected || cr) {
                    handed = true;
                    continue;
                }
                exp_head = expected;
                exp_batch = true;
                if (expected >= endw) {
                    stop = true;
                    continue;
                }
                const uint32_t bits = (uint32_t)(b9 >> (16 * k)) & 0xFFFFu;
                if (bits == 0u || ((nl2 >> (16 * k)) & 0xFFFFull) != 0ull) {
                    have_cand = false;
                    pos = expected;
                    handed = true;
                    expected = ~0ull;
                    continue;
                }
                record(expected);
                ++advanced;
                const int l9 = 16 * k + __builtin_ctz(bits);
                const uint32_t t9s = (uint32_t)__builtin_amdgcn_readlane((int)t9, l9);
                const uint64_t soff = cand - 40ull + (uint64_t)k * L0 + t9s + 1ull;
                const uint64_t nxt = soff + 4ull * S - 1ull;
                est_len = nxt - expected;
                expected = nxt;
                fbx = soff + 2ull * S - 17ull;
            }
            if (stop) break;
            if (expected != ~0ull) {
                if (expected > last_term) {
                    have_cand = false;
                    pos = fbx;
                    if (pos > last_term) pos = last_term;
                } else {
                    cand = expected;
                    fb = fbx > last_term ? last_term : fbx;
                    have_cand = true;
                }
                head_p = exp_head;
                cand_batch = exp_batch;
            }
            no_batch = handed;
            bat_fail = advanced ? 0u : bat_fail + 1u;
            bat_off = bat_fail >= 2u;
            continue;
        }
        no_batch = false;
        bool found = false, nb_have = false, have_head = false;
        uint32_t nb_reg = 0, ho = 15u;
        uint64_t p = 0;
        u32x4_t hd = u32x4_t{0u, 0u, 0u, 0u};
        if (WALK && have_cand) {
            have_cand = false;
            uint32_t c15 = 0, c14 = 0;
            const bool use_pf = pf_valid && cand >= pf_wb + 15ull && cand <= pf_wb + 79ull;
            pf_valid = false;
            if (use_pf || cand + 1009ull <= n) {
                if (use_pf) {
                    hd = pf;
                    ho = (uint32_t)(cand - pf_wb);
                } else
                    hd = *reinterpret_cast<const u32x4_unaligned *>(text + (cand - 15ull) + 16ull * lane);
                const uint64_t pred = cand + est_len;
                if (WALK_PF && est_len != 0ull && pred + 977ull <= n && cand < endw) {
                    pf_wb = pred - 47ull;
                    pf = *reinterpret_cast<const u32x4_unaligned *>(text + pf_wb + 16ull * lane);
                    pf_valid = true;
                }
                c15 = head_byte(hd, ho);
                c14 = head_byte(hd, ho - 1u);
                have_head = true;
            } else if (cand < n) {
                c15 = text[cand];
                c14 = text[cand - 1];
            } else if (cand == n && virt) {
                c15 = 0x0Au;
                c14 = text[n - 1];
            }
            if (c15 == 0x0Au && c14 != '\r') {
                found = true;
                p = cand;
            } else if (cand_batch) {
                cand_batch = false;
                rehead = true;
                found = true;
                have_head = false;
                p = head_p;
            } else {
                pos = fb;
                continue;
            }
        } else {
        const uint64_t a0 = pos & ~15ull;
        uint32_t any[U];
        u32x4_t v[U];
#pragma unroll
        for (int u = 0; u < U; ++u) {
            const uint64_t g0 = a0 + (uint64_t)u * 1024u + lane * 16u;
            uint32_t f = 0;
            v[u] = u32x4_t{0u, 0u, 0u, 0u};
            if (g0 + 16 <= n) {
                v[u] = __builtin_nontemporal_load(reinterpret_cast<const u32x4_t *>(text + g0));
                const uint32_t d[4] = {v[u].x, v[u].y, v[u].z, v[u].w};
#pragma unroll
                for (int q = 0; q < 4; ++q) {
                    const uint32_t t = d[q] ^ 0x0A0A0A0Au;
                    f |= (t - 0x01010101u) & ~t & 0x80808080u;
                }
            } else if (g0 <= n) {
                uint32_t d[4] = {0x20202020u, 0x20202020u, 0x20202020u, 0x20202020u};
                for (int j = 0; j < 16; ++j) {
                    const uint64_t g = g0 + j;
                    uint32_t ch = 0x20u;
                    if (g < n) ch = text[g];
                    else if (g == n && virt) ch = 0x0Au;
                    d[j >> 2] = (d[j >> 2] & ~(0xFFu << (8 * (j & 3)))) | (ch << (8 * (j & 3)));
                    if (ch == 0x0Au) f = 1u;
                }
                v[u] = u32x4_t{d[0], d[1], d[2], d[3]};
            }
            if (g0 + 16 <= pos) f = 0;
            any[u] = f;
        }
#pragma unroll
        for (int u = 0; u < U; ++u) {
            if (found) continue;
            unsigned long long b = __builtin_amdgcn_ballot_w64(any[u] != 0u);
            while (b != 0ull && !found) {
                const int l = __builtin_ctzll(b);
                b &= b - 1ull;
                const uint32_t x0 = (uint32_t)__builtin_amdgcn_readlane((int)v[u].x, l), x1 = (uint32_t)__builtin_amdgcn_readlane((int)v[u].y, l);
                const uint32_t x2 = (uint32_t)__builtin_amdgcn_readlane((int)v[u].z, l), x3 = (uint32_t)__builtin_amdgcn_readlane((int)v[u].w, l);
                uint32_t m = nl_mask4(x0) | (nl_mask4(x1) << 4) | (nl_mask4(x2) << 8) | (nl_mask4(x3) << 12);
                const uint64_t g0 = a0 + (uint64_t)u * 1024u + (uint64_t)l * 16u;
                if (g0 < pos) m &= ~((1u << (uint32_t)(pos - g0)) - 1u);
                if (m) {
                    found = true;
                    const uint32_t j = (uint32_t)__builtin_ctz(m);
                    p = g0 + j;
                    if (j < 15u && g0 + 16 <= n) {
                        const uint32_t k = j + 1u, dw = k >> 2;
                        const uint32_t xd = dw == 0u ? x0 : (dw == 1u ? x1 : (dw == 2u ? x2 : x3));
                        nb_reg = (xd >> (8u * (k & 3u))) & 0xFFu;
                        nb_have = true;
                    }
                }
            }
        }
        if (!found) {
            pos = a0 + (uint64_t)U * 1024u;
            continue;
        }
        }
        if (!rehead) {
            if (p >= endw) break;
            record(p);
        } else
            no_batch = true;
        rehead = false;
        bool hopped = false;
        if (WALK) {
            if (!have_head && p >= 15ull && p + 1009ull <= n) {
                hd = *reinterpret_cast<const u32x4_unaligned *>(text + (p - 15ull) + 16ull * lane);
                have_head = true;
            }
            if (have_head) {
                const uint64_t wb = p - (uint64_t)ho;
                const uint32_t nb = head_byte(hd, ho + 1u);
                const uint32_t l0 = 16u * lane;
                const uint32_t keep = l0 > ho ? 0xFFFFu : (l0 + 15u <= ho ? 0u : (0xFFFFu << (ho - l0 + 1u)) & 0xFFFFu);
                if (nb == '#' || nb == 0x0Au) {
                    pos = p + 1;
                    hopped = true;
                } else {
                    const uint32_t nlm = eq_mask16(hd, 0x0A0A0A0Au) & keep;
                    const unsigned long long nlb = __builtin_amdgcn_ballot_w64(nlm != 0u);
                    if (nlb != 0ull) {
                        const int l = __builtin_ctzll(nlb);
                        pos = wb + 16ull * (uint64_t)l + (uint64_t)__builtin_ctz((uint32_t)__builtin_amdgcn_readlane((int)nlm, l));
                        hopped = true;
                    } else {
                        const uint32_t tbm = eq_mask16(hd, 0x09090909u) & keep;
                        const uint32_t tc = (uint32_t)__popc(tbm);
                        const uint32_t incl = wave_scan_sum_dpp(tc, lane);
                        const uint32_t total = (uint32_t)__builtin_amdgcn_readlane((int)incl, 63);
                        if (total >= 9u) {
                            const uint32_t t8 = head_kth(tbm, incl - tc, 8u), t9 = head_kth(tbm, incl - tc, 9u);
                            const uint64_t soff = wb + t9 + 1ull;
                            const uint64_t lo = soff + 2ull * S - 17ull;
                            const bool gt = t9 - t8 == 3u && head_byte(hd, t8 + 1u) == 'G' && head_byte(hd, t8 + 2u) == 'T';
                            if (gt && soff + 4ull * S - 1ull <= last_term) {
                                cand = soff + 4ull * S - 1ull;
                                fb = lo;
                                have_cand = true;
                                est_len = cand - p;
                                head_p = p;
                                cand_batch = false;
                            } else {
                                pos = lo;
                            }
                            hopped = true;
                        }
                    }
                }
            }
        }
        if (!hopped) {
            uint32_t nb = 0x0Au;
            if (nb_have) nb = nb_reg;
            else if (p + 1 < n) nb = text[p + 1];
            pos = p + 1 + ((nb == '#' || nb == 0x0Au || nb == '\r') ? 0u : skip);
        }
        if (pos > last_term) pos = p + 1 > last_term ? p + 1 : last_term;
        if (have_cand && fb > last_term) fb = p + 1 > last_term ? p + 1 : last_term;
    }
    if (overflow && lane == 0) atomicAdd(&cnt->err_density, 1ull);
    if (lane < r_cnt) counts[r_first + lane] = cntv < INDEX_CAP ? cntv : INDEX_CAP;
}

__global__ __launch_bounds__(256) void k_compact_newlines(const uint32_t *__restrict__ slots,
                                                          const uint32_t *__restrict__ counts,
                                                          const uint32_t *__restrict__ prefix,
                                                          uint32_t n_regions, uint32_t *__restrict__ nl,
                                                          uint32_t max_lines)
{
    HHGT_WAVE_PRIO();
    uint32_t r = blockIdx.x * blockDim.x + threadIdx.x;
    if (r >= n_regions) return;
    uint32_t c = counts[r], p = prefix[r];
    const uint32_t *my = slots + (size_t)r * INDEX_CAP;
    for (uint32_t k = 0; k < c && p + k < max_lines; ++k) nl[p + k] = my[k];
}

__global__ __launch_bounds__(256) void k_parse_fixed(const uint8_t *__restrict__ text, uint64_t n,
                                                     const uint32_t *__restrict__ nl, const uint32_t *__restrict__ d_nlines,
                                                     uint32_t max_lines, const RegionFilter rfv, uint32_t S,
                                                     uint32_t *__restrict__ l_soff, uint32_t *__restrict__ l_lend,
                                                     uint32_t *__restrict__ l_pos, uint32_t *__restrict__ l_refalt,
                                                     uint32_t *__restrict__ l_flags, uint32_t *__restrict__ l_keep,
                                                     uint32_t *__restrict__ l_cnew, DevCounters *cnt, uint32_t hop_skip)
{
    HHGT_WAVE_PRIO();
    __shared__ uint32_t stage[256][17];
    const RegionFilter *rf = &rfv;
    const uint32_t i = blockIdx.x * blockDim.x + threadIdx.x;
    const uint32_t n_found = *d_nlines;
    const uint32_t n_lines = n_found < max_lines ? n_found : max_lines;
    if (i == 0) {
        cnt->n_lines = n_found;
        cnt->err_lines = n_found > max_lines ? (unsigned long long)(n_found - max_lines) : 0ull;
    }
    if (blockIdx.x * blockDim.x >= n_lines) {
        if (i < max_lines) l_keep[i] = l_cnew[i] = 0u;
        return;
    }
    uint32_t flags = 0;
    uint32_t s = 0, e = 0;
    bool staged = false;
    if (i < n_lines) {
        s = i ? nl[i - 1] + 1u : 0u;
        e = nl[i];
        staged = (uint64_t)s + 64ull <= n;
        if (staged) {
            u32x4_unaligned c[4];
#pragma unroll
            for (int k = 0; k < 4; ++k) c[k] = *reinterpret_cast<const u32x4_unaligned *>(text + s + 16 * k);
#pragma unroll
            for (int k = 0; k < 4; ++k) {
                stage[threadIdx.x][4 * k + 0] = c[k].x;
                stage[threadIdx.x][4 * k + 1] = c[k].y;
                stage[threadIdx.x][4 * k + 2] = c[k].z;
                stage[threadIdx.x][4 * k + 3] = c[k].w;
            }
        }
    }
    __syncthreads();
    const uint8_t *mine = reinterpret_cast<const uint8_t *>(stage[threadIdx.x]);
    auto rd = [&](uint32_t x) -> uint32_t { return (staged && x - s < 64u) ? (uint32_t)mine[x - s] : (uint32_t)text[x]; };
    uint32_t soff = 0, pos0 = 0, refalt = 0, gtidx = 0, stride = 0;
    if (i < n_lines) {
        if (e > s && rd(e - 1u) == '\r') --e;
        soff = e;
        if (e > s && rd(s) != '#') {
            flags = LF_RECORD;
            uint32_t fs[10];
            uint32_t nf = 0;
            uint32_t p = s;
            fs[0] = s;
            while (p < e && nf < 9) {
                if (rd(p) == '\t') fs[++nf] = p + 1;
                ++p;
            }
            bool bad = false;
            uint32_t fe[9];
#pragma unroll
            for (int k = 0; k < 9; ++k) fe[k] = (uint32_t)k < nf ? fs[k + 1] - 1u : e;
            if (nf < 7 || (S > 0 && nf < 9)) bad = true;
            if (!bad) {
                unsigned long long pos = 0;
                if (fe[1] == fs[1]) bad = true;
                for (uint32_t q = fs[1]; q < fe[1]; ++q) {
                    uint32_t c = rd(q);
                    if (c < '0' || c > '9') {
                        bad = true;
                        break;
                    }
                    pos = pos * 10ull + (c - '0');
                }
                bool in_region = true;
                if (!bad && rf->contig_len > 0) {
                    uint32_t cl = fe[0] - fs[0];
                    in_region = cl == (uint32_t)rf->contig_len;
                    for (uint32_t q = 0; in_region && q < cl; ++q)
                        in_region = rd(fs[0] + q) == (uint32_t)(uint8_t)rf->contig[q];
                    if (in_region && rf->has_range)
                        in_region = (long long)pos >= rf->beg && (long long)pos <= rf->end;
                }
                if (!bad) {
                    if (!in_region)
                        flags |= LF_DROP_REGION;
                    else {
                        uint32_t reflen = fe[3] - fs[3], altlen = fe[4] - fs[4];
                        uint32_t a = altlen >= 1 ? rd(fs[4]) : 0;
                        bool snp = reflen == 1 && altlen == 1 && (a == 'A' || a == 'C' || a == 'G' || a == 'T');
                        if (rf->keep_multi && reflen == 1 && altlen > 1 && (altlen & 1u)) {
                            snp = true;
                            for (uint32_t q = 0; snp && q < altlen; ++q) {
                                const uint32_t ch = rd(fs[4] + q);
                                snp = (q & 1u) ? ch == ',' : (ch == 'A' || ch == 'C' || ch == 'G' || ch == 'T');
                            }
                        }
                        if (!snp)
                            flags |= LF_DROP_FILTER;
                        else {
                            pos0 = (uint32_t)(pos - 1ull);
                            refalt = rd(fs[3]) | (a << 8);
                            if (S > 0) {
                                uint32_t q = fs[8], k = 0;
                                bool found = false;
                                while (q <= fe[8]) {
                                    uint32_t q2 = q;
                                    while (q2 < fe[8] && rd(q2) != ':') ++q2;
                                    if (q2 - q == 2 && rd(q) == 'G' && rd(q + 1u) == 'T') {
                                        found = true;
                                        break;
                                    }
                                    ++k;
                                    q = q2 + 1;
                                }
                                if (!found || k > 0xFFFu) bad = true;
                                gtidx = k;
                                soff = fs[9];
                                if (!bad) {
                                    flags |= LF_KEEP;
                                    if (k == 0 && fe[8] - fs[8] == 2 && e - soff == 4u * S - 1u) flags |= LF_FAST;
                                    else if (k == 0 && (e - soff + 1u) % S == 0u) {
                                        const uint32_t wd = (e - soff + 1u) / S;
                                        if (wd >= 5u && wd <= 8u) stride = wd;
                                    }
                                }
                            } else {
                                flags |= LF_KEEP;
                            }
                        }
                    }
                }
            }
            if (bad) flags = LF_RECORD | LF_MALFORMED;
            bool cnew = true;
            if (i > 0) {
                uint32_t ps = i > 1 ? nl[i - 2] + 1u : 0u;
                uint32_t pe = nl[i - 1];
                const bool pstaged = threadIdx.x > 0u && (uint64_t)ps + 64ull <= n;
                const uint8_t *prev = reinterpret_cast<const uint8_t *>(stage[threadIdx.x > 0u ? threadIdx.x - 1u : 0u]);
                auto rdp = [&](uint32_t x) -> uint32_t { return (pstaged && x - ps < 64u) ? (uint32_t)prev[x - ps] : (uint32_t)text[x]; };
                if (pe > ps && rdp(ps) != '#') {
                    uint32_t q = 0;
                    cnew = false;
                    for (;;) {
                        uint32_t a = fs[0] + q < e ? rd(fs[0] + q) : '\t';
                        uint32_t b = ps + q < pe ? rdp(ps + q) : '\t';
                        if (a != b) {
                            cnew = true;
                            break;
                        }
                        if (a == '\t') break;
                        ++q;
                    }
                }
            }
            if (cnew) flags |= LF_CHROM_NEW;
        }
    }
    if (hop_skip) {
        const uint32_t lane = threadIdx.x & 63u;
        const bool chk = (flags & LF_RECORD) && !(flags & (LF_KEEP | LF_MALFORMED));
        unsigned long long todo = __ballot(chk);
        while (todo != 0ull) {
            const int l = __builtin_ctzll(todo);
            todo &= todo - 1ull;
            const uint32_t ss = (uint32_t)__builtin_amdgcn_readlane((int)s, l), ee = (uint32_t)__builtin_amdgcn_readlane((int)e, l);
            const uint32_t hi = ee - ss < hop_skip ? ee : ss + hop_skip;
            uint32_t hit = 0;
            for (uint32_t x0 = ss + 16u * lane; x0 < hi; x0 += 8192u) {
                u32x4_t tv[8];
#pragma unroll
                for (int u = 0; u < 8; ++u) {
                    const uint32_t x = x0 + 1024u * (uint32_t)u;
                    tv[u] = u32x4_t{0u, 0u, 0u, 0u};
                    if (x < hi && (uint64_t)x + 16ull <= n) tv[u] = *reinterpret_cast<const u32x4_unaligned *>(text + x);
                }
#pragma unroll
                for (int u = 0; u < 8; ++u) {
                    const uint32_t x = x0 + 1024u * (uint32_t)u;
                    if (x >= hi) continue;
                    uint32_t d[4] = {tv[u].x, tv[u].y, tv[u].z, tv[u].w};
                    if ((uint64_t)x + 16ull > n)
                        for (uint32_t k = 0; k < 16u && (uint64_t)x + k < n; ++k) d[k >> 2] |= (uint32_t)text[x + k] << (8u * (k & 3u));
                    const uint32_t m = nl_mask4(d[0]) | (nl_mask4(d[1]) << 4) | (nl_mask4(d[2]) << 8) | (nl_mask4(d[3]) << 12);
                    hit |= hi - x >= 16u ? m : (m & ((1u << (hi - x)) - 1u));
                }
            }
            if (__ballot(hit != 0u) != 0ull && (int)lane == l) flags = (flags & LF_CHROM_NEW) | LF_RECORD | LF_MALFORMED;
        }
    }
    if (i < n_lines) {
        l_soff[i] = soff;
        l_lend[i] = e;
        l_pos[i] = pos0;
        l_refalt[i] = refalt | ((gtidx & 0xFFFu) << 16) | (stride << 28);
        l_flags[i] = flags;
        l_keep[i] = (flags & LF_KEEP) ? 1u : 0u;
        l_cnew[i] = (flags & LF_CHROM_NEW) ? 1u : 0u;
    } else if (i < max_lines) {
        l_keep[i] = l_cnew[i] = 0u;
    }
    __shared__ uint32_t s_stat[4];
    const uint32_t lane = threadIdx.x & 63u;
    if (threadIdx.x < 4u) s_stat[threadIdx.x] = 0u;
    __syncthreads();
    const uint32_t kinds[4] = {LF_RECORD, LF_DROP_REGION, LF_DROP_FILTER, LF_MALFORMED};
#pragma unroll
    for (int k = 0; k < 4; ++k) {
        const unsigned long long b = __ballot(flags & kinds[k]);
        if (lane == 0 && b) atomicAdd(&s_stat[k], (uint32_t)__popcll(b));
    }
    __syncthreads();
    if (threadIdx.x < 4u && s_stat[threadIdx.x]) {
        unsigned long long *dst = threadIdx.x == 0u ? &cnt->n_records : (threadIdx.x == 1u ? &cnt->n_drop_region : (threadIdx.x == 2u ? &cnt->n_drop_filter : &cnt->n_malformed));
        atomicAdd(dst, (unsigned long long)s_stat[threadIdx.x]);
    }
}

__global__ __launch_bounds__(256) void k_compact_kept(
    const uint8_t *__restrict__ text, uint64_t n, const uint32_t *__restrict__ nl, const uint32_t *__restrict__ d_nlines,
    uint32_t max_lines, const uint32_t *__restrict__ l_soff,
    const uint32_t *__restrict__ l_lend, const uint32_t *__restrict__ l_pos, const uint32_t *__restrict__ l_refalt,
    const uint32_t *__restrict__ l_flags, const uint32_t *__restrict__ l_kidx, const uint32_t *__restrict__ l_crun,
    uint32_t *__restrict__ k_soff, uint32_t *__restrict__ k_lend, uint32_t *__restrict__ k_meta,
    uint32_t *__restrict__ redo_list, uint32_t *__restrict__ redo_flag, uint64_t *__restrict__ run_first, uint8_t *__restrict__ run_names,
    uint32_t max_runs, const uint64_t *__restrict__ d_cursor, uint64_t v_capacity, uint32_t ring, uint32_t *__restrict__ d_start,
    uint32_t *__restrict__ d_stop, uint8_t *__restrict__ d_ref, uint8_t *__restrict__ d_alt, DevCounters *cnt, uint32_t strided)
{
    HHGT_WAVE_PRIO();
    const uint32_t i = blockIdx.x * blockDim.x + threadIdx.x;
    const uint32_t n_found = *d_nlines;
    const uint32_t n_lines = n_found < max_lines ? n_found : max_lines;
    if (i >= n_lines) return;
    const uint64_t v_base = *d_cursor;
    const uint32_t flags = l_flags[i];
    if (flags & LF_CHROM_NEW) {
        uint32_t rid = l_crun[i];
        if (rid < max_runs) {
            run_first[rid] = l_kidx[i];
            const uint32_t s0 = i ? nl[i - 1] + 1u : 0u;
            uint8_t *nm = run_names + (size_t)rid * 32u;
            uint32_t q = 0;
            for (; q < 31u && (uint64_t)s0 + q < n; ++q) {
                const uint8_t ch = text[s0 + q];
                if (ch == '\t' || ch == '\n') break;
                nm[q] = ch;
            }
            for (; q < 32u; ++q) nm[q] = 0;
        }
    }
    if (i == n_lines - 1) {
        cnt->n_kept = (unsigned long long)l_kidx[n_lines];
        cnt->n_chrom_runs = (unsigned long long)l_crun[n_lines];
    }
    const bool keep = (flags & LF_KEEP) != 0u;
    const bool slow = keep && !(flags & LF_FAST) && !(strided && (l_refalt[i < n_lines ? i : 0u] >> 28) != 0u);
    const unsigned long long sm = __ballot(slow);
    unsigned long long slot0 = 0ull;
    if (sm != 0ull) {
        const uint32_t lane = threadIdx.x & 63u;
        const int leader = __builtin_ctzll(sm);
        unsigned long long base = 0ull;
        if ((int)lane == leader) base = atomicAdd(&cnt->n_general, (unsigned long long)__popcll(sm));
        base = (unsigned long long)__shfl((long long)base, leader, 64);
        slot0 = base + (unsigned long long)__popcll(sm & ((1ull << lane) - 1ull));
    }
    if (!keep) return;
    const uint32_t k = l_kidx[i];
    uint64_t v = v_base + k;
    const uint32_t ra = l_refalt[i];
    k_soff[k] = l_soff[i];
    k_lend[k] = l_lend[i];
    k_meta[k] = (flags & LF_FAST) | ((ra >> 16) << 8);
    redo_flag[k] = 0u;
    if (slow) redo_list[slot0] = k;
    if (ring) v %= v_capacity;
    if (v < v_capacity) {
        uint32_t pos0 = l_pos[i];
        if (d_start) d_start[v] = pos0;
        if (d_stop) d_stop[v] = pos0 + 1u;
        if (d_ref) d_ref[v] = (uint8_t)(ra & 0xFFu);
        if (d_alt) d_alt[v] = (uint8_t)((ra >> 8) & 0xFFu);
    }
}

int index_mode_default()
{
    static const int m = [] {
        if (const char *e = getenv("HHGT_INDEX_MODE")) return atoi(e);
        if (const char *e = getenv("HHGT_INDEX_HOP")) return atoi(e) ? 2 : 0;
        return 2;
    }();
    return m < 0 ? 0 : (m > 2 ? 2 : m);
}

static uint32_t index_hop_skip(uint32_t min_line, int mode)
{
    if (mode < 0) mode = index_mode_default();
    return mode && min_line >= 1536u ? min_line - 16u : 0u;
}

int launch_index_newlines(const uint8_t *d_text, uint64_t n, uint32_t *d_slots, uint32_t *d_counts,
                          uint32_t n_regions, uint32_t min_line, uint32_t S, int mode, DevCounters *d_cnt, hipStream_t st)
{
    if (mode < 0) mode = index_mode_default();
    if (const uint32_t skip = index_hop_skip(min_line, mode)) {
        const bool walk = mode >= 2 && S > 0;
        const uint32_t k_walk = (n_regions + 8191u) / 8192u;
        uint32_t K = walk ? (k_walk < 6u ? 6u : k_walk) : 6u;
        K = K > 64u ? 64u : K;
#define HOP_LAUNCH(U, W)                                                                                                      \
    hipLaunchKernelGGL((k_index_hop<U, W>), dim3(((n_regions + K - 1) / K + 3) / 4), dim3(256), 0, st, d_text, n, d_slots, d_counts, \
                       n_regions, skip, S, d_cnt, K)
        if (min_line >= 4096u) {
            if (walk) HOP_LAUNCH(5, true);
            else HOP_LAUNCH(5, false);
        } else {
            if (walk) HOP_LAUNCH(3, true);
            else HOP_LAUNCH(3, false);
        }
#undef HOP_LAUNCH
        HIP_TRY(hipGetLastError());
        return HHGT_OK;
    }
    hipLaunchKernelGGL(k_index_newlines, dim3((n_regions + 3) / 4), dim3(256), 0, st, d_text, n, d_slots,
                       d_counts, n_regions, d_cnt);
    HIP_TRY(hipGetLastError());
    return HHGT_OK;
}

int launch_compact_newlines(const uint32_t *d_slots, const uint32_t *d_counts, const uint32_t *d_prefix,
                            uint32_t n_regions, uint32_t *d_nl, uint32_t max_lines, hipStream_t st)
{
    hipLaunchKernelGGL(k_compact_newlines, dim3((n_regions + 255) / 256), dim3(256), 0, st, d_slots, d_counts,
                       d_prefix, n_regions, d_nl, max_lines);
    HIP_TRY(hipGetLastError());
    return HHGT_OK;
}

int launch_parse_fixed(const uint8_t *d_text, uint64_t n, const uint32_t *d_nl, const uint32_t *d_nlines,
                       uint32_t max_lines, const RegionFilter &region, uint32_t S, uint32_t *l_soff, uint32_t *l_lend,
                       uint32_t *l_pos, uint32_t *l_refalt, uint32_t *l_flags, uint32_t *l_keep,
                       uint32_t *l_cnew, int mode, DevCounters *d_cnt, hipStream_t st)
{
    if (max_lines == 0) return HHGT_OK;
    if (mode < 0) mode = index_mode_default();
    uint32_t hop_skip = index_hop_skip(S ? 2u * S + 17u : 0u, mode);
    if (hop_skip && mode >= 2) hop_skip = 0xFFFFFFFFu;
    hipLaunchKernelGGL(k_parse_fixed, dim3((max_lines + 255) / 256), dim3(256), 0, st, d_text, n, d_nl, d_nlines,
                       max_lines, region, S, l_soff, l_lend, l_pos, l_refalt, l_flags, l_keep, l_cnew, d_cnt, hop_skip);
    HIP_TRY(hipGetLastError());
    return HHGT_OK;
}

int launch_compact_kept(const uint8_t *d_text, uint64_t n, const uint32_t *d_nl, const uint32_t *d_nlines, uint32_t max_lines,
                        const uint32_t *l_soff, const uint32_t *l_lend,
                        const uint32_t *l_pos, const uint32_t *l_refalt, const uint32_t *l_flags,
                        const uint32_t *l_kidx, const uint32_t *l_crun, uint32_t *k_soff, uint32_t *k_lend,
                        uint32_t *k_meta, uint32_t *redo_list, uint32_t *redo_flag, uint64_t *run_first, uint8_t *run_names,
                        uint32_t max_runs, const uint64_t *d_cursor, uint64_t v_capacity, uint32_t ring, uint32_t *d_start,
                        uint32_t *d_stop, uint8_t *d_ref, uint8_t *d_alt, DevCounters *d_cnt, bool strided, hipStream_t st)
{
    if (max_lines == 0) return HHGT_OK;
    hipLaunchKernelGGL(k_compact_kept, dim3((max_lines + 255) / 256), dim3(256), 0, st, d_text, n, d_nl, d_nlines, max_lines,
                       l_soff, l_lend, l_pos, l_refalt, l_flags, l_kidx, l_crun, k_soff, k_lend, k_meta, redo_list, redo_flag,
                       run_first, run_names, max_runs, d_cursor, v_capacity, ring, d_start, d_stop, d_ref, d_alt, d_cnt, strided ? 1u : 0u);
    HIP_TRY(hipGetLastError());
    return HHGT_OK;
}
```

haplohyped_varawareml_amd/csrc/scan.hip:

```cpp
#include "common.h"

#define SCAN_BLOCK 256
#define SCAN_ITEMS 8
#define SCAN_TILE (SCAN_BLOCK * SCAN_ITEMS)

__device__ __forceinline__ uint32_t wave_incl_scan(uint32_t v)
{
    const int lane = threadIdx.x & 63;
#pragma unroll
    for (int d = 1; d < 64; d <<= 1) {
        uint32_t t = __shfl_up(v, d, 64);
        if (lane >= d) v += t;
    }
    return v;
}

__device__ __forceinline__ uint32_t block_excl_scan(uint32_t v, uint32_t *total, uint32_t *sm )
{
    const int lane = threadIdx.x & 63, w = threadIdx.x >> 6;
    uint32_t inc = wave_incl_scan(v);
    if (lane == 63) sm[w] = inc;
    __syncthreads();
    uint32_t base = 0, tot = 0;
#pragma unroll
    for (int i = 0; i < SCAN_BLOCK / 64; ++i) {
        uint32_t x = sm[i];
        if (i < w) base += x;
        tot += x;
    }
    __syncthreads();
    *total = tot;
    return base + inc - v;
}

__global__ __launch_bounds__(SCAN_BLOCK) void k_scan_reduce(const uint32_t *__restrict__ in, uint64_t n,
                                                            uint32_t *__restrict__ partial)
{
    HHGT_WAVE_PRIO();
    __shared__ uint32_t sm[8];
    uint64_t base = (uint64_t)blockIdx.x * SCAN_TILE;
    uint32_t s = 0;
#pragma unroll
    for (int i = 0; i < SCAN_ITEMS; ++i) {
        uint64_t idx = base + (uint64_t)i * SCAN_BLOCK + threadIdx.x;
        if (idx < n) s += in[idx];
    }
    uint32_t tot;
    block_excl_scan(s, &tot, sm);
    if (threadIdx.x == 0) partial[blockIdx.x] = tot;
}

__global__ __launch_bounds__(SCAN_BLOCK) void k_scan_partials(uint32_t *partial, uint32_t nb)
{
    HHGT_WAVE_PRIO();
    __shared__ uint32_t sm[8];
    uint32_t carry = 0;
    for (uint32_t b0 = 0; b0 < nb; b0 += SCAN_BLOCK) {
        uint32_t i = b0 + threadIdx.x;
        uint32_t v = i < nb ? partial[i] : 0;
        uint32_t tot;
        uint32_t ex = block_excl_scan(v, &tot, sm);
        if (i < nb) partial[i] = carry + ex;
        carry += tot;
    }
    if (threadIdx.x == 0) partial[nb] = carry;
}

__global__ __launch_bounds__(SCAN_BLOCK) void k_scan_down(const uint32_t *__restrict__ in, uint64_t n,
                                                          const uint32_t *__restrict__ partial, uint32_t nb,
                                                          uint32_t *__restrict__ out)
{
    HHGT_WAVE_PRIO();
    __shared__ uint32_t sm[8];
    uint64_t base = (uint64_t)blockIdx.x * SCAN_TILE + (uint64_t)threadIdx.x * SCAN_ITEMS;
    uint32_t v[SCAN_ITEMS];
    uint32_t s = 0;
#pragma unroll
    for (int i = 0; i < SCAN_ITEMS; ++i) {
        uint64_t idx = base + i;
        v[i] = idx < n ? in[idx] : 0;
        s += v[i];
    }
    uint32_t tot;
    uint32_t ex = block_excl_scan(s, &tot, sm) + partial[blockIdx.x];
#pragma unroll
    for (int i = 0; i < SCAN_ITEMS; ++i) {
        uint64_t idx = base + i;
        if (idx < n) out[idx] = ex;
        ex += v[i];
    }
    if (blockIdx.x == 0 && threadIdx.x == 0) out[n] = partial[nb];
}

size_t scan_tmp_elems(uint64_t n) { return (size_t)((n + SCAN_TILE - 1) / SCAN_TILE) + 2; }

int launch_scan_exclusive_u32(const uint32_t *d_in, uint32_t *d_out, uint64_t n, uint32_t *d_tmp,
                              size_t tmp_elems, hipStream_t st)
{
    uint32_t nb = (uint32_t)((n + SCAN_TILE - 1) / SCAN_TILE);
    if (nb == 0) nb = 1;
    if (tmp_elems < (size_t)nb + 1) {
        hhgt_set_error("scan: tmp too small");
        return HHGT_ERR_ARG;
    }
    hipLaunchKernelGGL(k_scan_reduce, dim3(nb), dim3(SCAN_BLOCK), 0, st, d_in, n, d_tmp);
    hipLaunchKernelGGL(k_scan_partials, dim3(1), dim3(SCAN_BLOCK), 0, st, d_tmp, nb);
    hipLaunchKernelGGL(k_scan_down, dim3(nb), dim3(SCAN_BLOCK), 0, st, d_in, n, d_tmp, nb, d_out);
    HIP_TRY(hipGetLastError());
    return HHGT_OK;
}

template <int B>
__global__ __launch_bounds__(SCAN_BLOCK) void k_scan_reduce_n(const uint32_t *__restrict__ in0, const uint32_t *__restrict__ in1,
                                                              uint64_t n, uint32_t *__restrict__ partial, uint32_t nb)
{
    HHGT_WAVE_PRIO();
    __shared__ uint32_t sm[8];
    const uint32_t *ins[2] = {in0, in1};
    const uint64_t base = (uint64_t)blockIdx.x * SCAN_TILE;
#pragma unroll
    for (int b = 0; b < B; ++b) {
        uint32_t s = 0;
#pragma unroll
        for (int i = 0; i < SCAN_ITEMS; ++i) {
            const uint64_t idx = base + (uint64_t)i * SCAN_BLOCK + threadIdx.x;
            if (idx < n) s += ins[b][idx];
        }
        uint32_t tot;
        block_excl_scan(s, &tot, sm);
        if (threadIdx.x == 0) partial[(size_t)b * nb + blockIdx.x] = tot;
    }
}

template <int B>
__global__ __launch_bounds__(SCAN_BLOCK) void k_scan_down_n(const uint32_t *__restrict__ in0, const uint32_t *__restrict__ in1,
                                                            uint64_t n, const uint32_t *__restrict__ partial, uint32_t nb,
                                                            uint32_t *__restrict__ out0, uint32_t *__restrict__ out1)
{
    HHGT_WAVE_PRIO();
    __shared__ uint32_t sm[8];
    const uint32_t *ins[2] = {in0, in1};
    uint32_t *outs[2] = {out0, out1};
    const uint64_t base = (uint64_t)blockIdx.x * SCAN_TILE + (uint64_t)threadIdx.x * SCAN_ITEMS;
#pragma unroll
    for (int b = 0; b < B; ++b) {
        uint32_t pre = 0;
        for (uint32_t i = threadIdx.x; i < blockIdx.x; i += SCAN_BLOCK) pre += partial[(size_t)b * nb + i];
        uint32_t front;
        block_excl_scan(pre, &front, sm);
        uint32_t v[SCAN_ITEMS];
        uint32_t s = 0;
#pragma unroll
        for (int i = 0; i < SCAN_ITEMS; ++i) {
            const uint64_t idx = base + i;
            v[i] = idx < n ? ins[b][idx] : 0;
            s += v[i];
        }
        uint32_t tot;
        uint32_t ex = block_excl_scan(s, &tot, sm) + front;
#pragma unroll
        for (int i = 0; i < SCAN_ITEMS; ++i) {
            const uint64_t idx = base + i;
            if (idx < n) outs[b][idx] = ex;
            ex += v[i];
        }
        if (blockIdx.x == nb - 1 && threadIdx.x == 0) outs[b][n] = front + tot;
    }
}

#define SCAN_SHORT_MAX 2048u
int launch_scan_exclusive_u32_pair(const uint32_t *in_a, uint32_t *out_a, const uint32_t *in_b, uint32_t *out_b, uint64_t n,
                                   uint32_t *d_tmp, size_t tmp_elems, hipStream_t st)
{
    uint32_t nb = (uint32_t)((n + SCAN_TILE - 1) / SCAN_TILE);
    if (nb == 0) nb = 1;
    if (nb > SCAN_SHORT_MAX) {
        int rc = launch_scan_exclusive_u32(in_a, out_a, n, d_tmp, tmp_elems, st);
        if (rc == HHGT_OK && in_b) rc = launch_scan_exclusive_u32(in_b, out_b, n, d_tmp, tmp_elems, st);
        return rc;
    }
    if (tmp_elems < 2 * (size_t)nb) {
        hhgt_set_error("scan: tmp too small");
        return HHGT_ERR_ARG;
    }
    if (in_b) {
        hipLaunchKernelGGL(k_scan_reduce_n<2>, dim3(nb), dim3(SCAN_BLOCK), 0, st, in_a, in_b, n, d_tmp, nb);
        hipLaunchKernelGGL(k_scan_down_n<2>, dim3(nb), dim3(SCAN_BLOCK), 0, st, in_a, in_b, n, d_tmp, nb, out_a, out_b);
    } else {
        hipLaunchKernelGGL(k_scan_reduce_n<1>, dim3(nb), dim3(SCAN_BLOCK), 0, st, in_a, in_a, n, d_tmp, nb);
        hipLaunchKernelGGL(k_scan_down_n<1>, dim3(nb), dim3(SCAN_BLOCK), 0, st, in_a, in_a, n, d_tmp, nb, out_a, out_a);
    }
    HIP_TRY(hipGetLastError());
    return HHGT_OK;
}
```

Baseline: 151.6 million.

## Fuse scan passes into index/parse kernels, write results to mapped host memory

The newline-index and parse-fixed kernels now emit per-workgroup totals, so the compact kernels can compute exclusive prefixes themselves instead of running separate two-kernel scan passes over counts and keep/chrom-new flags. This removes several kernel launches and the full-size scanned per-line buffers whenever the workgroup count is under a threshold. The finish kernel can also write the result directly into a mapped pinned host buffer with a system-scope release store, replacing the device-to-host copy. The compress CU share is also raised. The cost is each compact workgroup summing preceding workgroup totals, plus reliance on mapped host memory being available.

```diff
diff --git a/haplohyped_varawareml_amd/csrc/api.hip b/haplohyped_varawareml_amd/csrc/api.hip
--- a/haplohyped_varawareml_amd/csrc/api.hip
+++ b/haplohyped_varawareml_amd/csrc/api.hip
@@ -109,7 +109,8 @@
     DevBuf *bufs[] = {&c->slots, &c->counts, &c->prefix, &c->nl, &c->scan_tmp, &c->l_soff, &c->l_lend, &c->l_pos,
                       &c->l_refalt, &c->l_flags, &c->l_keep, &c->l_kidx, &c->l_cnew, &c->l_crun, &c->k_soff,
                       &c->k_lend, &c->k_meta, &c->redo_list, &c->redo_flag, &c->run_first, &c->run_names,
-                      &c->counters, &c->cursor, &c->result, &c->dec_bad, &c->oh_ovl, &c->oh_lut, &c->crc_x2n};
+                      &c->counters, &c->cursor, &c->result, &c->dec_bad, &c->oh_ovl, &c->oh_lut, &c->crc_x2n, &c->idx_tot,
+                      &c->fix_tot};
     for (DevBuf *b : bufs) b->release();
     for (auto &w : c->cw) {
         DevBuf *wb[] = {&w.lz_scratch, &w.lz_csize, &w.lz_flags, &w.fr_bsize, &w.fr_csize, &w.fr_flags};
@@ -290,6 +291,7 @@
     return HHGT_OK;
 }
 
+template <bool HOST>
 __global__ void k_encode_finish(DevCounters *cnt, uint64_t *cursor, const uint64_t *__restrict__ run_first,
                                 const uint8_t *__restrict__ run_names, uint64_t v_capacity, hhgt_encode_result *res)
 {
@@ -314,14 +316,18 @@
         res->n_lines_over = cnt->err_lines;
         res->err_density = cnt->err_density;
         res->v_capacity = v_capacity;
-        res->done = 1u;
+        if (!HOST) res->done = 1u;
         res->reserved = cnt->n_other > 0xFFFFFFFFull ? 0xFFFFFFFFu : (uint32_t)cnt->n_other;
     }
     const uint64_t n_runs = cnt->n_chrom_runs;
     if (t < HHGT_RESULT_RUNS) res->run_first[t] = t < n_runs ? run_first[t] : 0ull;
     for (uint32_t q = t; q < HHGT_RESULT_RUNS * 32u; q += blockDim.x)
         res->run_names[q >> 5][q & 31u] = (q >> 5) < n_runs ? (char)run_names[q] : 0;
+    if (HOST) __threadfence_system();
     __syncthreads();
+    if (HOST && t == 0) {
+        __hip_atomic_store(&res->done, 1u, __ATOMIC_RELEASE, __HIP_MEMORY_SCOPE_SYSTEM);
+    }
     if (t < sizeof(DevCounters) / 8u) reinterpret_cast<unsigned long long *>(cnt)[t] = 0ull;
 }
 
@@ -350,13 +356,17 @@
 }
 
 static int encode_stage_index(hhgt_ctx *c, const uint8_t *text, uint64_t nbytes, uint32_t n_regions, uint32_t min_line, uint32_t S,
-                              DevCounters *cnt, hipStream_t st)
+                              DevCounters *cnt, bool fuse, hipStream_t st)
 {
     TRY(c->slots.ensure((size_t)n_regions * INDEX_CAP * 4));
     TRY(c->counts.ensure((size_t)n_regions * 4));
     TRY(c->prefix.ensure(((size_t)n_regions + 1) * 4));
     TRY(c->scan_tmp.ensure(2 * scan_tmp_elems(n_regions) * 4));
-    TRY(launch_index_newlines(text, nbytes, c->slots.as<uint32_t>(), c->counts.as<uint32_t>(), n_regions, min_line, S, c->index_mode, cnt, st));
+    TRY(c->idx_tot.ensure(INDEX_FUSE_MAX * 4));
+    c->idx_regions_per_wg = 0;
+    TRY(launch_index_newlines(text, nbytes, c->slots.as<uint32_t>(), c->counts.as<uint32_t>(), n_regions, min_line, S, c->index_mode, cnt,
+                              fuse ? c->idx_tot.as<uint32_t>() : nullptr, fuse ? &c->idx_regions_per_wg : nullptr, st));
+    if (c->idx_regions_per_wg) return HHGT_OK;
     TRY(launch_scan_exclusive_u32_pair(c->counts.as<uint32_t>(), c->prefix.as<uint32_t>(), nullptr, nullptr, n_regions,
                                        c->scan_tmp.as<uint32_t>(), c->scan_tmp.cap / 4, st));
     return HHGT_OK;
@@ -370,16 +380,29 @@
     const size_t nl4 = ((size_t)max_lines + 1) * 4;
     TRY(c->nl.ensure(nl4));
     TRY(c->scan_tmp.ensure(2 * scan_tmp_elems(max_lines) * 4));
-    DevBuf *per_line[] = {&c->l_soff, &c->l_lend, &c->l_pos, &c->l_refalt, &c->l_flags, &c->l_keep,
-                          &c->l_kidx, &c->l_cnew, &c->l_crun, &c->k_soff, &c->k_lend, &c->k_meta,
+    DevBuf *per_line[] = {&c->l_soff, &c->l_lend, &c->l_pos, &c->l_refalt, &c->l_flags, &c->k_soff, &c->k_lend, &c->k_meta,
                           &c->redo_list, &c->redo_flag};
     for (DevBuf *b : per_line) TRY(b->ensure(nl4));
+    const uint32_t n_fix_wg = (max_lines + 255u) / 256u;
+    const bool fix_fused = n_fix_wg <= FIXED_FUSE_MAX;
+    uint32_t *fix_tot = nullptr;
+    if (fix_fused) {
+        TRY(c->fix_tot.ensure((size_t)(n_fix_wg ? n_fix_wg : 1u) * 2 * 4));
+        fix_tot = c->fix_tot.as<uint32_t>();
+    } else {
+        DevBuf *scanned[] = {&c->l_keep, &c->l_kidx, &c->l_cnew, &c->l_crun};
+        for (DevBuf *b : scanned) TRY(b->ensure(nl4));
+    }
     TRY(c->run_first.ensure(MAX_CHROM_RUNS * 8));
     TRY(c->run_names.ensure(MAX_CHROM_RUNS * 32));
     {
         StageTimer t(c, st, HHGT_STAGE_INDEX);
-        TRY(launch_compact_newlines(c->slots.as<uint32_t>(), c->counts.as<uint32_t>(), c->prefix.as<uint32_t>(),
-                                    n_regions, c->nl.as<uint32_t>(), max_lines, st));
+        if (c->idx_regions_per_wg)
+            TRY(launch_compact_newlines_wg(c->slots.as<uint32_t>(), c->counts.as<uint32_t>(), c->idx_tot.as<uint32_t>(), n_regions,
+                                           c->idx_regions_per_wg, c->nl.as<uint32_t>(), max_lines, c->prefix.as<uint32_t>() + n_regions, st));
+        else
+            TRY(launch_compact_newlines(c->slots.as<uint32_t>(), c->counts.as<uint32_t>(), c->prefix.as<uint32_t>(),
+                                        n_regions, c->nl.as<uint32_t>(), max_lines, st));
         t.stop();
     }
     if (max_lines == 0) return HHGT_OK;
@@ -388,15 +411,16 @@
         TRY(launch_parse_fixed(text, nbytes, c->nl.as<uint32_t>(), d_nlines, max_lines, rf, L.S,
                                c->l_soff.as<uint32_t>(), c->l_lend.as<uint32_t>(), c->l_pos.as<uint32_t>(),
                                c->l_refalt.as<uint32_t>(), c->l_flags.as<uint32_t>(), c->l_keep.as<uint32_t>(),
-                               c->l_cnew.as<uint32_t>(), c->index_mode, cnt, st));
-        TRY(launch_scan_exclusive_u32_pair(c->l_keep.as<uint32_t>(), c->l_kidx.as<uint32_t>(), c->l_cnew.as<uint32_t>(),
-                                           c->l_crun.as<uint32_t>(), max_lines, c->scan_tmp.as<uint32_t>(), c->scan_tmp.cap / 4, st));
+                               c->l_cnew.as<uint32_t>(), c->index_mode, cnt, fix_tot, st));
+        if (!fix_fused)
+            TRY(launch_scan_exclusive_u32_pair(c->l_keep.as<uint32_t>(), c->l_kidx.as<uint32_t>(), c->l_cnew.as<uint32_t>(),
+                                               c->l_crun.as<uint32_t>(), max_lines, c->scan_tmp.as<uint32_t>(), c->scan_tmp.cap / 4, st));
         TRY(launch_compact_kept(text, nbytes, c->nl.as<uint32_t>(), d_nlines, max_lines, c->l_soff.as<uint32_t>(),
                                 c->l_lend.as<uint32_t>(), c->l_pos.as<uint32_t>(), c->l_refalt.as<uint32_t>(),
                                 c->l_flags.as<uint32_t>(), c->l_kidx.as<uint32_t>(), c->l_crun.as<uint32_t>(),
                                 c->k_soff.as<uint32_t>(), c->k_lend.as<uint32_t>(), c->k_meta.as<uint32_t>(),
                                 c->redo_list.as<uint32_t>(), c->redo_flag.as<uint32_t>(), c->run_first.as<uint64_t>(), c->run_names.as<uint8_t>(),
-                                MAX_CHROM_RUNS, d_cursor, L.v_capacity, L.ring, d_start, d_stop, d_ref, d_alt, cnt, d_P != nullptr, st));
+                                MAX_CHROM_RUNS, d_cursor, L.v_capacity, L.ring, d_start, d_stop, d_ref, d_alt, cnt, d_P != nullptr, fix_tot, st));
         t.stop();
     }
     if (L.S > 0) {
@@ -419,13 +443,18 @@
     return HHGT_OK;
 }
 
-static int encode_finish(hhgt_ctx *c, uint64_t *d_cursor, const LayoutDev &L, DevCounters *cnt, hipStream_t st)
+static int encode_finish(hhgt_ctx *c, uint64_t *d_cursor, const LayoutDev &L, DevCounters *cnt, hhgt_encode_result *d_host_result,
+                         hipStream_t st)
 {
     TRY(c->run_first.ensure(MAX_CHROM_RUNS * 8));
     TRY(c->run_names.ensure(MAX_CHROM_RUNS * 32));
     TRY(c->result.ensure(sizeof(hhgt_encode_result)));
-    hipLaunchKernelGGL(k_encode_finish, dim3(1), dim3(256), 0, st, cnt, d_cursor, c->run_first.as<uint64_t>(),
-                       c->run_names.as<uint8_t>(), L.ring ? 0ull : L.v_capacity, c->result.as<hhgt_encode_result>());
+    if (d_host_result)
+        hipLaunchKernelGGL(k_encode_finish<true>, dim3(1), dim3(256), 0, st, cnt, d_cursor, c->run_first.as<uint64_t>(),
+                           c->run_names.as<uint8_t>(), L.ring ? 0ull : L.v_capacity, d_host_result);
+    else
+        hipLaunchKernelGGL(k_encode_finish<false>, dim3(1), dim3(256), 0, st, cnt, d_cursor, c->run_first.as<uint64_t>(),
+                           c->run_names.as<uint8_t>(), L.ring ? 0ull : L.v_capacity, c->result.as<hhgt_encode_result>());
     HIP_TRY(hipGetLastError());
     return HHGT_OK;
 }
@@ -518,18 +547,23 @@
     if (nbytes) {
         {
             StageTimer t(c, st, HHGT_STAGE_INDEX);
-            TRY(encode_stage_index(c, text, nbytes, n_regions, L.S ? 2u * L.S + 17u : 0u, L.S, cnt, st));
+            TRY(encode_stage_index(c, text, nbytes, n_regions, L.S ? 2u * L.S + 17u : 0u, L.S, cnt, true, st));
             t.stop();
         }
         TRY(encode_stage_rest(c, text, nbytes, n_regions, max_lines, rf, L, d_cursor, d_G, planes ? d_P : nullptr, d_start, d_stop, d_ref,
                               d_alt, cnt, st));
     }
-    TRY(encode_finish(c, d_cursor, L, cnt, st));
+    hhgt_encode_result *d_host_result = nullptr;
+    if (h_result) {
+        void *dp = nullptr;
+        if (hipHostGetDevicePointer(&dp, h_result, 0) == hipSuccess && dp) d_host_result = static_cast<hhgt_encode_result *>(dp);
+        else (void)hipGetLastError();
+        h_result->done = 0u;
+    }
+    TRY(encode_finish(c, d_cursor, L, cnt, d_host_result, st));
     c->counters_clean = true;
-    if (h_result) {
-        h_result->done = 0u;
+    if (h_result && !d_host_result)
         HIP_TRY(hipMemcpyAsync(h_result, c->result.p, sizeof(hhgt_encode_result), hipMemcpyDeviceToHost, st));
-    }
     return HHGT_OK;
 }
 
@@ -636,7 +670,7 @@
     uint32_t n_lines = 0;
     {
         StageTimer t(c, st, HHGT_STAGE_INDEX);
-        TRY(encode_stage_index(c, text, nbytes, n_regions, L.S ? 2u * L.S + 17u : 0u, L.S, cnt, st));
+        TRY(encode_stage_index(c, text, nbytes, n_regions, L.S ? 2u * L.S + 17u : 0u, L.S, cnt, false, st));
         c->h_counters->n_lines = 0;
         c->h_counters->err_density = 0;
         HIP_TRY(hipMemcpyAsync(&c->h_counters->n_lines, c->prefix.as<uint32_t>() + n_regions, 4,
@@ -655,7 +689,7 @@
     if (n_lines == 0) return HHGT_OK;
     TRY(encode_stage_rest(c, text, nbytes, n_regions, n_lines, rf, L, c->cursor.as<uint64_t>(), d_G, nullptr, d_start, d_stop, d_ref,
                           d_alt, cnt, st));
-    TRY(encode_finish(c, c->cursor.as<uint64_t>(), L, cnt, st));
+    TRY(encode_finish(c, c->cursor.as<uint64_t>(), L, cnt, nullptr, st));
     c->counters_clean = true;
     hhgt_encode_result *hr = &c->h_result;
     hr->done = 0u;
@@ -885,9 +919,17 @@
         TRY(c->scan_tmp.ensure(2 * st_el * 4));
         const size_t nl4 = ((size_t)max_lines + 1) * 4;
         TRY(c->nl.ensure(nl4));
-        DevBuf *per_line[] = {&c->l_soff, &c->l_lend, &c->l_pos, &c->l_refalt, &c->l_flags, &c->l_keep, &c->l_kidx, &c->l_cnew, &c->l_crun,
-                              &c->k_soff, &c->k_lend, &c->k_meta, &c->redo_list, &c->redo_flag};
+        DevBuf *per_line[] = {&c->l_soff, &c->l_lend, &c->l_pos, &c->l_refalt, &c->l_flags, &c->k_soff, &c->k_lend, &c->k_meta, &c->redo_list,
+                              &c->redo_flag};
         for (DevBuf *b : per_line) TRY(b->ensure(nl4));
+        TRY(c->idx_tot.ensure(INDEX_FUSE_MAX * 4));
+        const uint32_t n_fix_wg = (max_lines + 255u) / 256u;
+        if (n_fix_wg <= FIXED_FUSE_MAX) {
+            TRY(c->fix_tot.ensure((size_t)(n_fix_wg ? n_fix_wg : 1u) * 2 * 4));
+        } else {
+            DevBuf *scanned[] = {&c->l_keep, &c->l_kidx, &c->l_cnew, &c->l_crun};
+            for (DevBuf *b : scanned) TRY(b->ensure(nl4));
+        }
         TRY(c->run_first.ensure(MAX_CHROM_RUNS * 8));
         TRY(c->run_names.ensure(MAX_CHROM_RUNS * 32));
         TRY(c->result.ensure(sizeof(hhgt_encode_result)));
@@ -904,7 +946,7 @@
         TRY(w.lz_csize.ensure((size_t)n_streams * 4));
         TRY(w.fr_bsize.ensure((size_t)n_chunks * nblocks * 4));
         TRY(w.fr_csize.ensure(((size_t)n_chunks + 1) * 8));
-        TRY(w.fr_flags.ensure((size_t)n_chunks * 4));
+            TRY(w.fr_flags.ensure((size_t)n_chunks * 4));
     }
     return HHGT_OK;
 }
@@ -935,7 +977,7 @@
         HIP_TRY(hipStreamCreateWithPriority(&st, hipStreamNonBlocking, hi));
     } else {
         const uint32_t n_cu = (uint32_t)c->prop.multiProcessorCount;
-        uint32_t use = n_cu >= 128u ? (n_cu * 3u / 4u) / 32u * 32u : n_cu;
+        uint32_t use = n_cu >= 128u ? (n_cu * 13u / 16u) / 16u * 16u : n_cu;
         if (const char *e = getenv("HHGT_COMPRESS_CUS")) {
             const int v = atoi(e);
             use = v <= 0 || (uint32_t)v >= n_cu ? n_cu : (uint32_t)v;
diff --git a/haplohyped_varawareml_amd/csrc/common.h b/haplohyped_varawareml_amd/csrc/common.h
--- a/haplohyped_varawareml_amd/csrc/common.h
+++ b/haplohyped_varawareml_amd/csrc/common.h
@@ -25,6 +25,64 @@
     const uint32_t t2 = (uint32_t)__builtin_amdgcn_readlane((int)x, 47) + t1;
     const uint32_t row = lane >> 4;
     return x + (row == 0u ? 0u : (row == 1u ? t0 : (row == 2u ? t1 : t2)));
+}
+
+#define SCAN_BLOCK 256
+__device__ __forceinline__ uint32_t wave_incl_scan(uint32_t v)
+{
+    const int lane = threadIdx.x & 63;
+#pragma unroll
+    for (int d = 1; d < 64; d <<= 1) {
+        uint32_t t = __shfl_up(v, d, 64);
+        if (lane >= d) v += t;
+    }
+    return v;
+}
+
+__device__ __forceinline__ uint32_t block_excl_scan(uint32_t v, uint32_t *total, uint32_t *sm )
+{
+    const int lane = threadIdx.x & 63, w = threadIdx.x >> 6;
+    uint32_t inc = wave_incl_scan(v);
+    if (lane == 63) sm[w] = inc;
+    __syncthreads();
+    uint32_t base = 0, tot = 0;
+#pragma unroll
+    for (int i = 0; i < SCAN_BLOCK / 64; ++i) {
+        uint32_t x = sm[i];
+        if (i < w) base += x;
+        tot += x;
+    }
+    __syncthreads();
+    *total = tot;
+    return base + inc - v;
+}
+
+__device__ __forceinline__ void block_excl_scan2(uint32_t va, uint32_t vb, uint32_t *ex_a, uint32_t *ex_b, uint32_t *tot_a,
+                                                 uint32_t *tot_b, uint32_t *sm)
+{
+    const int lane = threadIdx.x & 63, w = threadIdx.x >> 6;
+    const uint32_t ia = wave_incl_scan(va), ib = wave_incl_scan(vb);
+    if (lane == 63) {
+        sm[w] = ia;
+        sm[4 + w] = ib;
+    }
+    __syncthreads();
+    uint32_t ba = 0, bb = 0, ta = 0, tb = 0;
+#pragma unroll
+    for (int i = 0; i < SCAN_BLOCK / 64; ++i) {
+        const uint32_t xa = sm[i], xb = sm[4 + i];
+        if (i < w) {
+            ba += xa;
+            bb += xb;
+        }
+        ta += xa;
+        tb += xb;
+    }
+    __syncthreads();
+    *tot_a = ta;
+    *tot_b = tb;
+    *ex_a = ba + ia - va;
+    *ex_b = bb + ib - vb;
 }
 #endif
 
@@ -135,6 +193,8 @@
     int device = 0;
     hipDeviceProp_t prop;
     DevBuf slots, counts, prefix, nl, scan_tmp;
+    DevBuf idx_tot, fix_tot;
+    uint32_t idx_regions_per_wg = 0;
     DevBuf l_soff, l_lend, l_pos, l_refalt, l_flags, l_keep, l_kidx, l_cnew, l_crun;
     DevBuf k_soff, k_lend, k_meta, redo_list, redo_flag, run_first, run_names;
     DevBuf counters;
@@ -183,22 +243,28 @@
                                    uint32_t *d_tmp, size_t tmp_elems, hipStream_t st);
 size_t scan_tmp_elems(uint64_t n);
 
+#define INDEX_FUSE_MAX 8192u
+#define FIXED_FUSE_MAX 4096u
 int launch_index_newlines(const uint8_t *d_text, uint64_t n, uint32_t *d_slots, uint32_t *d_counts,
-                          uint32_t n_regions, uint32_t min_line, uint32_t S, int mode, DevCounters *d_cnt, hipStream_t st);
+                          uint32_t n_regions, uint32_t min_line, uint32_t S, int mode, DevCounters *d_cnt, uint32_t *d_wg_tot,
+                          uint32_t *regions_per_wg, hipStream_t st);
+int launch_compact_newlines_wg(const uint32_t *d_slots, const uint32_t *d_counts, const uint32_t *d_wg_tot, uint32_t n_regions,
+                               uint32_t regions_per_wg, uint32_t *d_nl, uint32_t max_lines, uint32_t *d_nlines, hipStream_t st);
 int index_mode_default();
 int launch_compact_newlines(const uint32_t *d_slots, const uint32_t *d_counts, const uint32_t *d_prefix,
                             uint32_t n_regions, uint32_t *d_nl, uint32_t max_lines, hipStream_t st);
 int launch_parse_fixed(const uint8_t *d_text, uint64_t n, const uint32_t *d_nl, const uint32_t *d_nlines,
                        uint32_t max_lines, const RegionFilter &region, uint32_t S, uint32_t *l_soff, uint32_t *l_lend,
                        uint32_t *l_pos, uint32_t *l_refalt, uint32_t *l_flags, uint32_t *l_keep,
-                       uint32_t *l_cnew, int mode, DevCounters *d_cnt, hipStream_t st);
+                       uint32_t *l_cnew, int mode, DevCounters *d_cnt, uint32_t *d_wg_tot, hipStream_t st);
 int launch_compact_kept(const uint8_t *d_text, uint64_t n, const uint32_t *d_nl, const uint32_t *d_nlines, uint32_t max_lines,
                         const uint32_t *l_soff, const uint32_t *l_lend,
                         const uint32_t *l_pos, const uint32_t *l_refalt, const uint32_t *l_flags,
                         const uint32_t *l_kidx, const uint32_t *l_crun, uint32_t *k_soff, uint32_t *k_lend,
                         uint32_t *k_meta, uint32_t *redo_list, uint32_t *redo_flag, uint64_t *run_first, uint8_t *run_names,
                         uint32_t max_runs, const uint64_t *d_cursor, uint64_t v_capacity, uint32_t ring, uint32_t *d_start,
-                        uint32_t *d_stop, uint8_t *d_ref, uint8_t *d_alt, DevCounters *d_cnt, bool strided, hipStream_t st);
+                        uint32_t *d_stop, uint8_t *d_ref, uint8_t *d_alt, DevCounters *d_cnt, bool strided, const uint32_t *d_wg_tot,
+                        hipStream_t st);
 
 int launch_encode_tiles(const uint8_t *d_text, uint64_t n, const uint32_t *k_soff, const uint32_t *k_meta,
                         uint32_t n_lines_bound, const uint64_t *d_cursor, LayoutDev lay, int8_t *d_G,
diff --git a/haplohyped_varawareml_amd/csrc/index.hip b/haplohyped_varawareml_amd/csrc/index.hip
--- a/haplohyped_varawareml_amd/csrc/index.hip
+++ b/haplohyped_varawareml_amd/csrc/index.hip
@@ -106,15 +106,14 @@
 #define WALK_PF 0
 #endif
 template <int U, bool WALK>
-__global__ __launch_bounds__(256) void k_index_hop(const uint8_t *__restrict__ text, uint64_t n, uint32_t *__restrict__ slots,
+__device__ __forceinline__ uint32_t index_hop_wave(const uint8_t *__restrict__ text, uint64_t n, uint32_t *__restrict__ slots,
                                                    uint32_t *__restrict__ counts, uint32_t n_regions, uint32_t skip, uint32_t S,
                                                    DevCounters *cnt, uint32_t HOP_K)
 {
-    HHGT_WAVE_PRIO();
     const uint32_t lane = threadIdx.x & 63u;
     const uint32_t w = (uint32_t)__builtin_amdgcn_readfirstlane((int)(blockIdx.x * 4u + (threadIdx.x >> 6)));
     const uint32_t r_first = w * HOP_K;
-    if (r_first >= n_regions) return;
+    if (r_first >= n_regions) return 0u;
     const uint32_t r_cnt = n_regions - r_first < HOP_K ? n_regions - r_first : HOP_K;
     const bool virt = n > 0 && text[n - 1] != '\n';
     const uint64_t beg = (uint64_t)r_first * INDEX_REGION;
@@ -415,7 +414,23 @@
         if (have_cand && fb > last_term) fb = p + 1 > last_term ? p + 1 : last_term;
     }
     if (overflow && lane == 0) atomicAdd(&cnt->err_density, 1ull);
-    if (lane < r_cnt) counts[r_first + lane] = cntv < INDEX_CAP ? cntv : INDEX_CAP;
+    const uint32_t stored = lane < r_cnt ? (cntv < INDEX_CAP ? cntv : INDEX_CAP) : 0u;
+    if (lane < r_cnt) counts[r_first + lane] = stored;
+    return (uint32_t)__builtin_amdgcn_readlane((int)wave_scan_sum_dpp(stored, lane), 63);
+}
+
+template <int U, bool WALK>
+__global__ __launch_bounds__(256) void k_index_hop(const uint8_t *__restrict__ text, uint64_t n, uint32_t *__restrict__ slots,
+                                                   uint32_t *__restrict__ counts, uint32_t n_regions, uint32_t skip, uint32_t S,
+                                                   DevCounters *cnt, uint32_t HOP_K, uint32_t *__restrict__ wg_tot)
+{
+    HHGT_WAVE_PRIO();
+    __shared__ uint32_t s_tot[4];
+    const uint32_t t = index_hop_wave<U, WALK>(text, n, slots, counts, n_regions, skip, S, cnt, HOP_K);
+    if (!wg_tot) return;
+    if ((threadIdx.x & 63u) == 0u) s_tot[threadIdx.x >> 6] = t;
+    __syncthreads();
+    if (threadIdx.x == 0u) wg_tot[blockIdx.x] = s_tot[0] + s_tot[1] + s_tot[2] + s_tot[3];
 }
 
 __global__ __launch_bounds__(256) void k_compact_newlines(const uint32_t *__restrict__ slots,
@@ -432,13 +447,34 @@
     for (uint32_t k = 0; k < c && p + k < max_lines; ++k) nl[p + k] = my[k];
 }
 
+__global__ __launch_bounds__(256) void k_compact_newlines_wg(const uint32_t *__restrict__ slots, const uint32_t *__restrict__ counts,
+                                                             const uint32_t *__restrict__ wg_tot, uint32_t n_regions, uint32_t per_wg,
+                                                             uint32_t *__restrict__ nl, uint32_t max_lines, uint32_t *__restrict__ d_nlines)
+{
+    HHGT_WAVE_PRIO();
+    __shared__ uint32_t sm[8];
+    uint32_t pre = 0;
+    for (uint32_t i = threadIdx.x; i < blockIdx.x; i += 256u) pre += wg_tot[i];
+    uint32_t front;
+    block_excl_scan(pre, &front, sm);
+    const uint32_t r = blockIdx.x * per_wg + threadIdx.x;
+    const bool mine = threadIdx.x < per_wg && r < n_regions;
+    const uint32_t c = mine ? counts[r] : 0u;
+    uint32_t tot;
+    const uint32_t p = block_excl_scan(c, &tot, sm) + front;
+    if (blockIdx.x == gridDim.x - 1u && threadIdx.x == 0u) *d_nlines = front + tot;
+    const uint32_t *my = slots + (size_t)r * INDEX_CAP;
+    for (uint32_t k = 0; k < c && p + k < max_lines; ++k) nl[p + k] = my[k];
+}
+
 __global__ __launch_bounds__(256) void k_parse_fixed(const uint8_t *__restrict__ text, uint64_t n,
                                                      const uint32_t *__restrict__ nl, const uint32_t *__restrict__ d_nlines,
                                                      uint32_t max_lines, const RegionFilter rfv, uint32_t S,
                                                      uint32_t *__restrict__ l_soff, uint32_t *__restrict__ l_lend,
                                                      uint32_t *__restrict__ l_pos, uint32_t *__restrict__ l_refalt,
                                                      uint32_t *__restrict__ l_flags, uint32_t *__restrict__ l_keep,
-                                                     uint32_t *__restrict__ l_cnew, DevCounters *cnt, uint32_t hop_skip)
+                                                     uint32_t *__restrict__ l_cnew, DevCounters *cnt, uint32_t hop_skip,
+                                                     uint32_t *__restrict__ wg_tot)
 {
     HHGT_WAVE_PRIO();
     __shared__ uint32_t stage[256][17];
@@ -451,7 +487,10 @@
         cnt->err_lines = n_found > max_lines ? (unsigned long long)(n_found - max_lines) : 0ull;
     }
     if (blockIdx.x * blockDim.x >= n_lines) {
-        if (i < max_lines) l_keep[i] = l_cnew[i] = 0u;
+        if (wg_tot) {
+            if (threadIdx.x < 2u) wg_tot[threadIdx.x * gridDim.x + blockIdx.x] = 0u;
+        } else if (i < max_lines)
+            l_keep[i] = l_cnew[i] = 0u;
         return;
     }
     uint32_t flags = 0;
@@ -630,28 +669,32 @@
         l_pos[i] = pos0;
         l_refalt[i] = refalt | ((gtidx & 0xFFFu) << 16) | (stride << 28);
         l_flags[i] = flags;
-        l_keep[i] = (flags & LF_KEEP) ? 1u : 0u;
-        l_cnew[i] = (flags & LF_CHROM_NEW) ? 1u : 0u;
-    } else if (i < max_lines) {
+        if (!wg_tot) {
+            l_keep[i] = (flags & LF_KEEP) ? 1u : 0u;
+            l_cnew[i] = (flags & LF_CHROM_NEW) ? 1u : 0u;
+        }
+    } else if (i < max_lines && !wg_tot) {
         l_keep[i] = l_cnew[i] = 0u;
     }
-    __shared__ uint32_t s_stat[4];
+    __shared__ uint32_t s_stat[6];
     const uint32_t lane = threadIdx.x & 63u;
-    if (threadIdx.x < 4u) s_stat[threadIdx.x] = 0u;
+    if (threadIdx.x < 6u) s_stat[threadIdx.x] = 0u;
     __syncthreads();
-    const uint32_t kinds[4] = {LF_RECORD, LF_DROP_REGION, LF_DROP_FILTER, LF_MALFORMED};
-#pragma unroll
-    for (int k = 0; k < 4; ++k) {
+    const uint32_t kinds[6] = {LF_RECORD, LF_DROP_REGION, LF_DROP_FILTER, LF_MALFORMED, LF_KEEP, LF_CHROM_NEW};
+#pragma unroll
+    for (int k = 0; k < 6; ++k) {
         const unsigned long long b = __ballot(flags & kinds[k]);
         if (lane == 0 && b) atomicAdd(&s_stat[k], (uint32_t)__popcll(b));
     }
     __syncthreads();
+    if (wg_tot && threadIdx.x < 2u) wg_tot[threadIdx.x * gridDim.x + blockIdx.x] = s_stat[4u + threadIdx.x];
     if (threadIdx.x < 4u && s_stat[threadIdx.x]) {
         unsigned long long *dst = threadIdx.x == 0u ? &cnt->n_records : (threadIdx.x == 1u ? &cnt->n_drop_region : (threadIdx.x == 2u ? &cnt->n_drop_filter : &cnt->n_malformed));
         atomicAdd(dst, (unsigned long long)s_stat[threadIdx.x]);
     }
 }
 
+template <bool FUSED>
 __global__ __launch_bounds__(256) void k_compact_kept(
     const uint8_t *__restrict__ text, uint64_t n, const uint32_t *__restrict__ nl, const uint32_t *__restrict__ d_nlines,
     uint32_t max_lines, const uint32_t *__restrict__ l_soff,
@@ -666,13 +709,32 @@
     const uint32_t i = blockIdx.x * blockDim.x + threadIdx.x;
     const uint32_t n_found = *d_nlines;
     const uint32_t n_lines = n_found < max_lines ? n_found : max_lines;
-    if (i >= n_lines) return;
+    uint32_t flags = 0, kidx = 0, crun = 0;
+    if (FUSED) {
+        __shared__ uint32_t sm[8];
+        if (blockIdx.x * blockDim.x >= n_lines) return;
+        uint32_t pk = 0, pc = 0, fk, fc, tk, tc;
+        for (uint32_t j = threadIdx.x; j < blockIdx.x; j += 256u) {
+            pk += l_kidx[j];
+            pc += l_kidx[gridDim.x + j];
+        }
+        block_excl_scan2(pk, pc, &kidx, &crun, &fk, &fc, sm);
+        if (i < n_lines) flags = l_flags[i];
+        block_excl_scan2((flags & LF_KEEP) ? 1u : 0u, (flags & LF_CHROM_NEW) ? 1u : 0u, &kidx, &crun, &tk, &tc, sm);
+        kidx += fk;
+        crun += fc;
+        if (i >= n_lines) return;
+    } else {
+        if (i >= n_lines) return;
+        flags = l_flags[i];
+        kidx = l_kidx[i];
+        crun = (flags & LF_CHROM_NEW) ? l_crun[i] : 0u;
+    }
     const uint64_t v_base = *d_cursor;
-    const uint32_t flags = l_flags[i];
     if (flags & LF_CHROM_NEW) {
-        uint32_t rid = l_crun[i];
+        uint32_t rid = crun;
         if (rid < max_runs) {
-            run_first[rid] = l_kidx[i];
+            run_first[rid] = kidx;
             const uint32_t s0 = i ? nl[i - 1] + 1u : 0u;
             uint8_t *nm = run_names + (size_t)rid * 32u;
             uint32_t q = 0;
@@ -685,8 +747,13 @@
         }
     }
     if (i == n_lines - 1) {
-        cnt->n_kept = (unsigned long long)l_kidx[n_lines];
-        cnt->n_chrom_runs = (unsigned long long)l_crun[n_lines];
+        if (FUSED) {
+            cnt->n_kept = (unsigned long long)(kidx + ((flags & LF_KEEP) ? 1u : 0u));
+            cnt->n_chrom_runs = (unsigned long long)(crun + ((flags & LF_CHROM_NEW) ? 1u : 0u));
+        } else {
+            cnt->n_kept = (unsigned long long)l_kidx[n_lines];
+            cnt->n_chrom_runs = (unsigned long long)l_crun[n_lines];
+        }
     }
     const bool keep = (flags & LF_KEEP) != 0u;
     const bool slow = keep && !(flags & LF_FAST) && !(strided && (l_refalt[i < n_lines ? i : 0u] >> 28) != 0u);
@@ -701,7 +768,7 @@
         slot0 = base + (unsigned long long)__popcll(sm & ((1ull << lane) - 1ull));
     }
     if (!keep) return;
-    const uint32_t k = l_kidx[i];
+    const uint32_t k = kidx;
     uint64_t v = v_base + k;
     const uint32_t ra = l_refalt[i];
     k_soff[k] = l_soff[i];
@@ -736,17 +803,22 @@
 }
 
 int launch_index_newlines(const uint8_t *d_text, uint64_t n, uint32_t *d_slots, uint32_t *d_counts,
-                          uint32_t n_regions, uint32_t min_line, uint32_t S, int mode, DevCounters *d_cnt, hipStream_t st)
+                          uint32_t n_regions, uint32_t min_line, uint32_t S, int mode, DevCounters *d_cnt, uint32_t *d_wg_tot,
+                          uint32_t *regions_per_wg, hipStream_t st)
 {
     if (mode < 0) mode = index_mode_default();
+    if (regions_per_wg) *regions_per_wg = 0;
     if (const uint32_t skip = index_hop_skip(min_line, mode)) {
         const bool walk = mode >= 2 && S > 0;
         const uint32_t k_walk = (n_regions + 8191u) / 8192u;
         uint32_t K = walk ? (k_walk < 6u ? 6u : k_walk) : 6u;
         K = K > 64u ? 64u : K;
+        const uint32_t n_wg = ((n_regions + K - 1) / K + 3) / 4;
+        uint32_t *wg_tot = d_wg_tot && regions_per_wg && n_wg <= INDEX_FUSE_MAX ? d_wg_tot : nullptr;
+        if (wg_tot) *regions_per_wg = 4u * K;
 #define HOP_LAUNCH(U, W)                                                                                                      \
-    hipLaunchKernelGGL((k_index_hop<U, W>), dim3(((n_regions + K - 1) / K + 3) / 4), dim3(256), 0, st, d_text, n, d_slots, d_counts, \
-                       n_regions, skip, S, d_cnt, K)
+    hipLaunchKernelGGL((k_index_hop<U, W>), dim3(n_wg), dim3(256), 0, st, d_text, n, d_slots, d_counts, n_regions, skip, S, d_cnt, K, \
+                       wg_tot)
         if (min_line >= 4096u) {
             if (walk) HOP_LAUNCH(5, true);
             else HOP_LAUNCH(5, false);
@@ -773,17 +845,26 @@
     return HHGT_OK;
 }
 
+int launch_compact_newlines_wg(const uint32_t *d_slots, const uint32_t *d_counts, const uint32_t *d_wg_tot, uint32_t n_regions,
+                               uint32_t regions_per_wg, uint32_t *d_nl, uint32_t max_lines, uint32_t *d_nlines, hipStream_t st)
+{
+    hipLaunchKernelGGL(k_compact_newlines_wg, dim3((n_regions + regions_per_wg - 1) / regions_per_wg), dim3(256), 0, st, d_slots,
+                       d_counts, d_wg_tot, n_regions, regions_per_wg, d_nl, max_lines, d_nlines);
+    HIP_TRY(hipGetLastError());
+    return HHGT_OK;
+}
+
 int launch_parse_fixed(const uint8_t *d_text, uint64_t n, const uint32_t *d_nl, const uint32_t *d_nlines,
                        uint32_t max_lines, const RegionFilter &region, uint32_t S, uint32_t *l_soff, uint32_t *l_lend,
                        uint32_t *l_pos, uint32_t *l_refalt, uint32_t *l_flags, uint32_t *l_keep,
-                       uint32_t *l_cnew, int mode, DevCounters *d_cnt, hipStream_t st)
+                       uint32_t *l_cnew, int mode, DevCounters *d_cnt, uint32_t *d_wg_tot, hipStream_t st)
 {
     if (max_lines == 0) return HHGT_OK;
     if (mode < 0) mode = index_mode_default();
     uint32_t hop_skip = index_hop_skip(S ? 2u * S + 17u : 0u, mode);
     if (hop_skip && mode >= 2) hop_skip = 0xFFFFFFFFu;
     hipLaunchKernelGGL(k_parse_fixed, dim3((max_lines + 255) / 256), dim3(256), 0, st, d_text, n, d_nl, d_nlines,
-                       max_lines, region, S, l_soff, l_lend, l_pos, l_refalt, l_flags, l_keep, l_cnew, d_cnt, hop_skip);
+                       max_lines, region, S, l_soff, l_lend, l_pos, l_refalt, l_flags, l_keep, l_cnew, d_cnt, hop_skip, d_wg_tot);
     HIP_TRY(hipGetLastError());
     return HHGT_OK;
 }
@@ -794,12 +875,18 @@
                         const uint32_t *l_kidx, const uint32_t *l_crun, uint32_t *k_soff, uint32_t *k_lend,
                         uint32_t *k_meta, uint32_t *redo_list, uint32_t *redo_flag, uint64_t *run_first, uint8_t *run_names,
                         uint32_t max_runs, const uint64_t *d_cursor, uint64_t v_capacity, uint32_t ring, uint32_t *d_start,
-                        uint32_t *d_stop, uint8_t *d_ref, uint8_t *d_alt, DevCounters *d_cnt, bool strided, hipStream_t st)
+                        uint32_t *d_stop, uint8_t *d_ref, uint8_t *d_alt, DevCounters *d_cnt, bool strided, const uint32_t *d_wg_tot,
+                        hipStream_t st)
 {
     if (max_lines == 0) return HHGT_OK;
-    hipLaunchKernelGGL(k_compact_kept, dim3((max_lines + 255) / 256), dim3(256), 0, st, d_text, n, d_nl, d_nlines, max_lines,
-                       l_soff, l_lend, l_pos, l_refalt, l_flags, l_kidx, l_crun, k_soff, k_lend, k_meta, redo_list, redo_flag,
-                       run_first, run_names, max_runs, d_cursor, v_capacity, ring, d_start, d_stop, d_ref, d_alt, d_cnt, strided ? 1u : 0u);
+    if (d_wg_tot)
+        hipLaunchKernelGGL(k_compact_kept<true>, dim3((max_lines + 255) / 256), dim3(256), 0, st, d_text, n, d_nl, d_nlines, max_lines,
+                           l_soff, l_lend, l_pos, l_refalt, l_flags, d_wg_tot, nullptr, k_soff, k_lend, k_meta, redo_list, redo_flag,
+                           run_first, run_names, max_runs, d_cursor, v_capacity, ring, d_start, d_stop, d_ref, d_alt, d_cnt, strided ? 1u : 0u);
+    else
+        hipLaunchKernelGGL(k_compact_kept<false>, dim3((max_lines + 255) / 256), dim3(256), 0, st, d_text, n, d_nl, d_nlines, max_lines,
+                           l_soff, l_lend, l_pos, l_refalt, l_flags, l_kidx, l_crun, k_soff, k_lend, k_meta, redo_list, redo_flag,
+                           run_first, run_names, max_runs, d_cursor, v_capacity, ring, d_start, d_stop, d_ref, d_alt, d_cnt, strided ? 1u : 0u);
     HIP_TRY(hipGetLastError());
     return HHGT_OK;
 }
diff --git a/haplohyped_varawareml_amd/csrc/scan.hip b/haplohyped_varawareml_amd/csrc/scan.hip
--- a/haplohyped_varawareml_amd/csrc/scan.hip
+++ b/haplohyped_varawareml_amd/csrc/scan.hip
@@ -1,37 +1,8 @@
 #include "common.h"
 
-#define SCAN_BLOCK 256
 #define SCAN_ITEMS 8
 #define SCAN_TILE (SCAN_BLOCK * SCAN_ITEMS)
 
-__device__ __forceinline__ uint32_t wave_incl_scan(uint32_t v)
-{
-    const int lane = threadIdx.x & 63;
-#pragma unroll
-    for (int d = 1; d < 64; d <<= 1) {
-        uint32_t t = __shfl_up(v, d, 64);
-        if (lane >= d) v += t;
-    }
-    return v;
-}
-
-__device__ __forceinline__ uint32_t block_excl_scan(uint32_t v, uint32_t *total, uint32_t *sm )
-{
-    const int lane = threadIdx.x & 63, w = threadIdx.x >> 6;
-    uint32_t inc = wave_incl_scan(v);
-    if (lane == 63) sm[w] = inc;
-    __syncthreads();
-    uint32_t base = 0, tot = 0;
-#pragma unroll
-    for (int i = 0; i < SCAN_BLOCK / 64; ++i) {
-        uint32_t x = sm[i];
-        if (i < w) base += x;
-        tot += x;
-    }
-    __syncthreads();
-    *total = tot;
-    return base + inc - v;
-}
 
 __global__ __launch_bounds__(SCAN_BLOCK) void k_scan_reduce(const uint32_t *__restrict__ in, uint64_t n,
                                                             uint32_t *__restrict__ partial)
```

Result: no change. 151.8 million (median of 3 runs) (+0.1%).
